# tamthuc1995/ImageRestoration-Development-Unrolling

Measured on AMD Instinct MI355X. Metric: MPix/sec + PSNR@σ=25, 10-stage GGTV-GGLR on 256×256 patches, 1/2/4/8 GPU, higher is better.
Workload: dtype f32; 1 GPU; MultiScaleGraphFilter (image-domain GGTV-GGLR, v13 feature CNN) G=32 F=3 C=96, S=10 stages, 256x256 RGB sigma=25, weights: trained fixture; global_batch=64, per_gpu_batch=64, image=256x256x3, parallelism=batch-sharded x1, no collective in the data path

## Files before the change

imagerestoration-development-unrolling_amd/_native.py:

```python
from __future__ import annotations

import ctypes
import os
from ctypes import c_int, c_int64, c_void_p

HERE = os.path.dirname(os.path.abspath(__file__))
LIB_PATH = os.environ.get("GRR_LIB", os.path.join(HERE, "libgrr.so"))


class NativeUnavailable(RuntimeError):
    """libgrr.so could not be loaded (build it with build_native.py)."""


class GrrError(RuntimeError):

    def __init__(self, fn: str, status: int, msg: str):
        super().__init__(f"{fn} failed (status {status}): {msg}")
        self.status = status


STATUS_NAMES = {0: "GRR_OK", 1: "GRR_ERR_INVALID_ARG", 2: "GRR_ERR_SHAPE", 3: "GRR_ERR_UNSUPPORTED", 4: "GRR_ERR_HIP"}


class Stencil(ctypes.Structure):
    _fields_ = [("p01", c_void_p), ("p02a", c_void_p), ("p02b", c_void_p), ("p03", c_void_p)]


P = c_void_p
I = c_int
L = c_int64
Fl = ctypes.c_float

SIGNATURES = {
    "grr_version": [],
    "grr_last_error": [],
    "grr_set_kernel_variant": [I],
    "grr_lnb_set_phases": [I],
    "grr_lnb_rep_fused": [I, I, I, I],
    "grr_set_scratch_allocator": [P, P, P],
    "grr_release_scratch": [],
    "grr_scratch_bytes": [],
    "grr_neighbor_table": [P, I, I, P],
    "grr_stream_copy": [P, P, L, P],
    "grr_edge_weights": [P, L, P, P, P, I, I, I, I, I, P],
    "grr_gtv_pair_weights": [P, P, I, I, I, I, P],
    "grr_edge_weights_block": [P, L, I, P, I, P, P, P, P, I, I, I, I, I, P],
    "grr_pool2": [P, P, I, I, I, I, P],
    "grr_system_half": [P, P, P, Stencil, Stencil, P, P, P, I, I, I, I, I, P],
    "grr_gtv_rhs_half": [P, P, Stencil, I, P, P, I, I, I, I, I, P],
    "grr_gtv_rhs_full": [P, P, P, Stencil, I, P, P, P, P, P, P, I, I, I, I, I, P],
    "grr_gtv_rhs_full_rep": [P, I, P, I, P, Stencil, I, P, P, P, P, P, P, I, I, I, I, I, P],
    "grr_system_step": [P, P, P, P, P, P, Stencil, Stencil, P, P, P, P, P, P, P, P, P, I, I, I, I, I, P],
    "grr_system_step2": [P, P, P, P, P, P, Stencil, Stencil, P, P, P, P, Stencil, Stencil, P, P, P, P, P, P, P, P,
                         P, P, P, I, I, I, I, I, P],
    "grr_system_first_pair": [P, P, P, I, P, P, P, Stencil, Stencil, P, P, P, P, P, P, Stencil, Stencil, P, P, P, P, P,
                              P, P, P, P, I, I, I, I, I, P],
    "grr_system_step2_train": [P, P, P, P, P, P, Stencil, Stencil, P, P, P, P, Stencil, Stencil, P, P, P, P, P, P,
                               P, P, P, P, P, P, I, I, I, I, I, P],
    "grr_glr_stage": [P, P, P, P, Stencil, P, P, P, P, P, I, I, I, I, I, P],
    "grr_conv1x1": [P, P, P, I, I, I, L, P],
    "grr_conv1x1_workspace_bytes": [I, I],
    "grr_conv1x1_ws": [P, P, P, P, I, I, I, L, P],
    "grr_conv2x2s2": [P, P, P, I, I, I, I, I, P],
    "grr_conv3x3_embed_supported": [I, I],
    "grr_conv3x3_embed": [P, P, P, I, I, I, I, I, P],
    "grr_conv3x3_embed_bwd_w_workspace_bytes": [I, I, I, I, I],
    "grr_conv3x3_embed_bwd_w": [P, P, P, P, I, I, I, I, I, P],
    "grr_conv3x3_embed_bwd_x": [P, P, P, I, I, I, I, I, P],
    "grr_convt2x2s2_workspace_bytes": [I, I, I, I, I],
    "grr_convt2x2s2": [P, P, P, P, I, I, I, I, I, P],
    "grr_conv1x1_cat2_supported": [I, I, I, L],
    "grr_conv1x1_cat2_workspace_bytes": [I, I, I],
    "grr_conv1x1_cat2": [P, P, P, P, P, I, I, I, I, L, P],
    "grr_ffn_workspace_bytes": [I, I, I, I, I],
    "grr_ffn_forward": [P, P, P, P, P, P, P, P, I, I, I, I, I, P],
    "grr_wgrad_workspace_bytes": [I, I, I, L],
    "grr_wgrad_set_tiles": [I],
    "grr_wgrad": [P, P, P, P, I, I, I, L, P],
    "grr_lnb_workspace_bytes": [I, I, I, I, I],
    "grr_lnb_forward": [P, P, P, P, P, P, P, P, I, I, I, I, I, P],
    "grr_lnb_forward_keep": [P, P, P, P, P, P, P, P, I, I, I, I, I, P],
    "grr_lnb_forward_c8": [P, P, P, P, P, P, P, P, I, I, I, I, I, I, P],
    "grr_c8_convert": [P, P, I, I, I, I, I, P],
    "grr_feature_edges_supported": [I, I, I, I, I],
    "grr_feature_edges_workspace_bytes": [I],
    "grr_feature_edges": [P, I, P, P, P, P, P, P, P, I, I, I, I, I, I, P],
    "grr_lnb_fused": [I, I],
    "grr_lnb_fused_workspace_bytes": [I, I],
    "grr_lnb_set_fused": [I],
    "grr_dw3_ring_check": [I],
    "grr_repeat_graphs": [P, P, I, I, I, L, P],
    "grr_lnb_forward_rep": [P, I, I, P, P, P, P, P, P, P, P, I, I, I, I, P],
    "grr_neighbor_gather": [P, P, I, I, I, I, P],
    "grr_normalize_features": [P, P, P, I, I, I, I, I, P],
    "grr_stats_conv": [P, Stencil, I, P, I, I, I, I, I, P],
    "grr_glr_op_l_norm": [P, P, P, I, I, I, I, I, P],
    "grr_gtv_op_c": [P, P, Stencil, P, I, I, I, I, I, P],
    "grr_gtv_op_c_transpose": [P, P, Stencil, P, P, I, I, I, I, I, P],
    "grr_neighbor_gather_bwd": [P, P, I, I, I, I, P],
    "grr_normalize_features_bwd": [P, P, P, P, P, I, I, I, I, I, P],
    "grr_stats_conv_bwd": [P, Stencil, I, P, P, P, I, I, I, I, I, P],
    "grr_glr_op_l_norm_bwd": [P, P, P, P, P, I, I, I, I, I, P],
    "grr_gtv_op_c_bwd": [P, P, Stencil, P, P, P, P, P, I, I, I, I, I, P],
    "grr_gtv_op_c_transpose_bwd": [P, P, Stencil, P, P, P, P, P, P, I, I, I, I, I, P],
    "grr_bwd_stencil": [P, P, I, P, I, P, I, I, I, I, I, P],
    "grr_bwd_tapgrad": [P, P, I, P, P, I, I, I, I, I, P],
    "grr_bwd_padj2": [P, P, P, P, P, P, P, I, I, I, I, I, P],
    "grr_bwd_glr": [P, P, P, P, Fl, P, P, P, P, I, I, I, I, I, P],
    "grr_bwd_pair": [P, P, P, P, Fl, P, P, P, P, I, I, I, I, I, P],
    "grr_bwd_prox": [P, P, P, P, P, Fl, P, P, P, P, P, I, I, I, I, I, P],
    "grr_bwd_set_term_rows": [I],
    "grr_bwd_set_term_tail": [I],
    "grr_bwd_set_term_acc_max_w": [I],
    "grr_lnb_set_bwd_ring": [I],
    "grr_bwd_term_fused": [I, P, P, P, P, P, P, Fl, P, P, P, P, P, I, I, I, I, I, P],
    "grr_bwd_term_acc_supported": [I, I, I, I],
    "grr_bwd_term_fused_acc": [I, P, P, P, P, P, P, Fl, P, P, P, P, P, I, I, I, I, I, P],
    "grr_bwd_pair_weights": [P, P, P, I, I, I, I, P],
    "grr_bwd_edge_weights": [P, L, P, P, P, P, L, P, I, I, I, I, I, P],
    "grr_bwd_graph_dot": [P, P, Fl, P, I, I, I, I, I, P],
    "grr_bwd_lincomb": [P, P, P, P, P, I, I, I, I, I, I, P],
    "grr_bwd_cg_glue": [P, P, P, P, P, P, P, P, P, P, P, P, P, P, P, P, P, P, I, I, I, I, I, P],
    "grr_bwd_cg_glue_pool": [P, P, P, P, P, P, P, P, P, P, P, P, P, P, P, P, P, P, P, I, I, I, I, I, P],
    "grr_bwd_unpool2_acc": [P, P, I, I, I, I, P],
    "grr_conv2x2s2_bwd_data": [P, P, P, I, I, I, I, I, P],
    "grr_interleave2x2": [P, P, I, I, I, I, P],
    "grr_lnb_norm": [P, P, P, P, I, I, L, P],
    "grr_lnb_norm_bwd": [P, P, P, P, P, P, I, I, L, P],
    "grr_lnb_norm_bwd_skip": [P, P, P, P, P, P, P, P, P, I, I, L, P],
    "grr_dwconv3": [P, P, P, I, I, I, I, P],
    "grr_dwconv3_bwd": [P, P, P, P, P, I, I, I, I, P],
    "grr_lnb_gate": [P, P, P, P, I, I, L, P],
    "grr_lnb_gate_bwd_scaled": [P, P, P, P, P, I, I, L, P],
    "grr_lnb_gate_dw3_bwd": [P, P, P, P, P, P, P, P, I, I, I, I, P],
    "grr_lnb_dw3_gate": [P, P, P, I, I, I, I, P],
    "grr_ffn_dw3_gate": [P, P, P, I, I, I, I, P],
    "grr_ffn_gate_dw3_bwd": [P, P, P, P, P, P, P, I, I, I, I, P],
    "grr_win_edge_weights": [P, L, P, P, I, P, P, I, I, I, I, I, P],
    "grr_win_solver": [I, P, I, P, P, P, P, P, P, P, P, P, P, P, P, I, P, P, I, I, I, I, I, P],
    "grr_win_mix": [P, P, P, P, I, I, I, I, I, P],
    "grr_win_pair_weights": [P, P, I, P, I, I, I, I, P],
    "grr_win_bwd_stencil": [P, P, I, P, I, P, I, I, I, I, I, P],
    "grr_win_bwd_tapgrad": [P, P, I, P, P, I, I, I, I, I, P],
    "grr_win_bwd_glr": [P, P, P, P, I, P, Fl, P, P, P, P, P, I, I, I, I, I, P],
    "grr_win_bwd_gtv": [P, P, P, P, I, I, P, P, Fl, P, P, P, P, P, P, I, I, I, I, I, P],
    "grr_win_bwd_gather": [P, P, P, I, P, P, I, I, I, I, I, P],
    "grr_win_bwd_gather_fused": [P, P, P, P, I, I, I, P, P, P, P, I, I, I, I, I, P],
    "grr_win_bwd_edge_weights": [P, L, P, P, P, P, I, P, L, P, I, I, I, I, I, P],
    "grr_win_bwd_mix": [P, P, P, P, P, I, I, I, I, I, P],
    "grr_image_io_supported": [I, I, I],
    "grr_tile_gather": [P, I, I, I, I, P, I, I, I, P, P],
    "grr_tile_scatter": [P, P, I, I, I, P, I, I, I, I, P],
    "grr_u8_sse": [P, P, L, P, P],
}
_RESTYPES = {"grr_version": c_int, "grr_last_error": ctypes.c_char_p, "grr_lnb_workspace_bytes": c_int64,
             "grr_conv1x1_workspace_bytes": c_int64, "grr_wgrad_workspace_bytes": c_int64,
             "grr_ffn_workspace_bytes": c_int64, "grr_scratch_bytes": c_int64,
             "grr_lnb_fused_workspace_bytes": c_int64, "grr_feature_edges_workspace_bytes": c_int64,
             "grr_conv3x3_embed_bwd_w_workspace_bytes": c_int64, "grr_conv1x1_cat2_workspace_bytes": c_int64, "grr_convt2x2s2_workspace_bytes": c_int64}

_lib = None


def load() -> ctypes.CDLL:
    global _lib
    if _lib is not None:
        return _lib
    if not os.path.exists(LIB_PATH):
        raise NativeUnavailable(
            f"{LIB_PATH} not found: build it with `python imagerestoration-development-unrolling_amd/build_native.py`")
    try:
        lib = ctypes.CDLL(LIB_PATH)
    except OSError as e:
        raise NativeUnavailable(f"cannot load {LIB_PATH}: {e}") from e
    for name, argtypes in SIGNATURES.items():
        fn = getattr(lib, name)
        fn.argtypes = argtypes
        fn.restype = _RESTYPES.get(name, c_int)
    _register_scratch_allocator(lib)
    _lib = lib
    return lib


_SCRATCH_ALLOC_FN = ctypes.CFUNCTYPE(c_void_p, ctypes.c_uint64, c_int, c_void_p, c_void_p)
_SCRATCH_FREE_FN = ctypes.CFUNCTYPE(None, c_void_p, c_int, c_void_p, c_void_p)


def _scratch_alloc(nbytes, device, stream, _ctx):
    try:
        import torch
        return int(torch.cuda.caching_allocator_alloc(int(nbytes), device, int(stream or 0)))
    except Exception:
        return None


def _scratch_free(ptr, _device, _stream, _ctx):
    try:
        import torch
        torch.cuda.caching_allocator_delete(int(ptr))
    except Exception:
        pass


_scratch_cbs = (_SCRATCH_ALLOC_FN(_scratch_alloc), _SCRATCH_FREE_FN(_scratch_free))


def _register_scratch_allocator(lib) -> None:
    st = lib.grr_set_scratch_allocator(ctypes.cast(_scratch_cbs[0], c_void_p), ctypes.cast(_scratch_cbs[1], c_void_p),
                                       None)
    if st != 0:
        raise NativeUnavailable(f"grr_set_scratch_allocator failed: {lib.grr_last_error()!r}")


def release_scratch() -> None:
    import torch
    torch.cuda.synchronize()
    call("grr_release_scratch")


def call(name: str, *args) -> None:
    lib = load()
    st = getattr(lib, name)(*args)
    if st != 0:
        msg = lib.grr_last_error()
        raise GrrError(name, st, (msg or b"").decode(errors="replace"))
```

imagerestoration-development-unrolling_amd/csrc/feature_ops.hip:

```cpp
#include "grr_common.h"

namespace grr {

typedef float f32x16 __attribute__((ext_vector_type(16)));

constexpr int GT = 256;
constexpr int BM = 128, BN = 128, BK = 16;
constexpr int APAD = BM + 2;
constexpr int BPAD = BN + 4;

enum { LD_PLAIN = 0, LD_LN = 1, LD_IM2COL = 2 };
enum { EP_STORE = 0, EP_SKIP = 1 };

struct GemmArgs {
  const float* x;
  const float* wt;
  const float* ln_sd;
  const float* ln_w;
  const float* res;
  const float* skip;
  float* out;
  int K, M;
  int64_t P;
  int Hin, Win, Wo;
// ... 766 lines not shown
}

int64_t grr_conv1x1_cat2_workspace_bytes(int Ka, int Kb, int M) {
  if (Ka < 1 || Kb < 1) return 0;
  return grr_conv1x1_workspace_bytes(Ka + Kb, M);
}

grr_status grr_conv1x1_cat2(const float* xa, const float* xb, const float* wt, float* out, void* workspace, int B,
                            int Ka, int Kb, int M, int64_t P, void* stream) {
  clear_error();
  GRR_REQUIRE(xa && xb && wt && out && workspace && B > 0 && Ka > 0 && Kb > 0 && M > 0 && P > 0, GRR_ERR_INVALID_ARG,
              "grr_conv1x1_cat2: bad args");
  GRR_REQUIRE(out != xa && out != xb, GRR_ERR_INVALID_ARG, "grr_conv1x1_cat2: out aliases an input");
  GRR_REQUIRE(((uintptr_t)workspace & 255) == 0, GRR_ERR_INVALID_ARG, "grr_conv1x1_cat2: workspace not 256-B aligned");
  GRR_REQUIRE(grr_conv1x1_cat2_supported(Ka, Kb, M, P), GRR_ERR_UNSUPPORTED,
              "grr_conv1x1_cat2: Ka=%d (a multiple of 16), Kb=%d, M=%d, P=%lld not supported", Ka, Kb, M, (long long)P);
  hipStream_t s = (hipStream_t)stream;
  const int K = Ka + Kb, KS = (K + 15) / 16, nch = (M + X3_MCH - 1) / X3_MCH;
  uint16_t* frag = (uint16_t*)workspace;
  const int64_t nf = (int64_t)nch * x3_chunk_bytes(KS) / 2;
  hipLaunchKernelGGL(x3_pack_kernel, dim3((unsigned)std::min<int64_t>((nf + 255) / 256, 1 << 16)), dim3(256), 0, s,
                     wt, nullptr, frag, M, K, KS, nch);
  grr_status st = launch_status("grr_conv1x1_cat2/pack");
  if (st != GRR_OK) return st;
  if (K > 128)
    return launch_x3k<X3K_STORE, true>(xa, frag, out, B, K, M, P, s, "grr_conv1x1_cat2", nullptr, nullptr, nullptr, xb,
                                       Ka);
  return launch_x3<false, true>(xa, frag, out, B, K, M, P, s, "grr_conv1x1_cat2", xb, Ka);
}

grr_status grr_conv2x2s2(const float* x, const float* wt, float* out, int B, int K, int M, int H, int W,
                         void* stream) {
  clear_error();
  GRR_REQUIRE(x && wt && out && B > 0 && K > 0 && M > 0 && H > 1 && W > 1, GRR_ERR_INVALID_ARG,
              "grr_conv2x2s2: bad args");
  GemmArgs a{};
  a.x = x; a.wt = wt; a.out = out; a.K = 4 * K; a.M = M; a.P = (int64_t)(H / 2) * (W / 2);
  a.Hin = H; a.Win = W; a.Wo = W / 2;
  return launch_gemm<LD_IM2COL, EP_STORE>(a, B, (hipStream_t)stream, "grr_conv2x2s2");
}

}

namespace grr {

struct FfnLayout {
  int64_t sd, h, g, f1, f2, total;
  int KS1, nch1, KS2, nch2;
};
static int64_t a64(int64_t n) { return (n + 63) / 64 * 64; }
static FfnLayout ffn_layout(int B, int C, int hid, int64_t P) {
  FfnLayout L{};
  L.KS1 = (C + 15) / 16; L.nch1 = (2 * hid + 31) / 32;
  L.KS2 = (hid + 15) / 16; L.nch2 = (C + 31) / 32;
  L.sd = 0;
  L.h = a64((int64_t)B * P);
  L.g = L.h + a64((int64_t)B * 2 * hid * P);
  L.f1 = L.g + a64((int64_t)B * hid * P);
  L.f2 = L.f1 + a64((int64_t)L.nch1 * x3_chunk_bytes(L.KS1) / 4);
  L.total = L.f2 + a64((int64_t)L.nch2 * x3_chunk_bytes(L.KS2) / 4);
  return L;
}

template <bool FFN>
static grr_status block_x3_forward(const float* x, const float* ln_w, const float* w_in, const float* w_dw,
                                   const float* w_out, const float* skip, float* out, float* ws, int B, int C,
                                   int hid, int H, int W, hipStream_t s) {
  const int64_t P = (int64_t)H * W;
  const FfnLayout L = ffn_layout(B, C, hid, P);
  float* sd = ws + L.sd;
  float* hbuf = ws + L.h;
  float* gbuf = ws + L.g;
  uint16_t* f1 = reinterpret_cast<uint16_t*>(ws + L.f1);
  uint16_t* f2 = reinterpret_cast<uint16_t*>(ws + L.f2);
  auto pack = [&](const float* w, const float* lw, uint16_t* frag, int M, int K, int KS, int nch) {
    const int64_t nf = (int64_t)nch * x3_chunk_bytes(KS) / 2;
    hipLaunchKernelGGL(x3_pack_kernel, dim3((unsigned)std::min<int64_t>((nf + 255) / 256, 1 << 16)), dim3(256), 0, s,
                       w, lw, frag, M, K, KS, nch);
    return launch_status("grr_ffn_forward/pack");
  };
  grr_status st = pack(w_in, ln_w, f1, 2 * hid, C, L.KS1, L.nch1);
  if (st != GRR_OK) return st;
  st = pack(w_out, nullptr, f2, C, hid, L.KS2, L.nch2);
  if (st != GRR_OK) return st;
  if (C <= 128) {
    st = launch_x3<true>(x, f1, hbuf, B, C, 2 * hid, P, s, "grr_ffn_forward/w_in");
  } else {
    GRR_REQUIRE((int64_t)B * ((P + 63) / 64) < (1ll << 31), GRR_ERR_UNSUPPORTED, "grr_ffn_forward: grid too large");
    hipLaunchKernelGGL(ln_stats_kernel, dim3((unsigned)((int64_t)B * ((P + 63) / 64))), dim3(64 * LN_G), 0, s, x, sd,
                       B, C, P);
    st = launch_status("grr_ffn_forward/ln_stats");
    if (st != GRR_OK) return st;
    st = launch_x3k<X3K_LN>(x, f1, hbuf, B, C, 2 * hid, P, s, "grr_ffn_forward/w_in", sd);
  }
  if (st != GRR_OK) return st;
  const int tx = (W + DT - 1) / DT, ty = (H + DT - 1) / DT;
  const uint64_t nb = (uint64_t)B * hid * tx * ty;
  GRR_REQUIRE(nb < (1ull << 31), GRR_ERR_UNSUPPORTED, "grr_ffn_forward: grid too large");
  hipLaunchKernelGGL(dw_gate_kernel<FFN>, dim3((unsigned)nb), dim3(256), 0, s, hbuf, w_dw, gbuf, hid, H, W, tx, ty,
                     (uint32_t)nb);
  st = launch_status("grr_ffn_forward/dw_gate");
  if (st != GRR_OK) return st;
  return launch_x3k<X3K_SKIP>(gbuf, f2, out, B, hid, C, P, s, "grr_ffn_forward/w_out", nullptr, x, skip);
}

}

extern "C" {

int64_t grr_lnb_workspace_bytes(int B, int C, int hid, int H, int W) {
  if (B <= 0 || C <= 0 || hid <= 0 || H <= 0 || W <= 0) return 0;
  const int64_t f = C <= 128 ? grr::lnb_mfma_workspace_floats(B, C, hid, H, W)
                             : grr::ffn_layout(B, C, hid, (int64_t)H * W).total;
  return f * (int64_t)sizeof(float);
}

int64_t grr_lnb_fused_workspace_bytes(int C, int hid) {
  if (!grr::lnb_fused(C, hid)) return 0;
  return grr::fused_pack_floats(C, hid) * (int64_t)sizeof(float);
}

grr_status grr_lnb_forward(const float* x, const float* ln_w, const float* w1, const float* wdw, const float* w2,
                           const float* skip, float* out, void* workspace, int B, int C, int hid, int H, int W,
                           void* stream) {
  grr::clear_error();
  GRR_REQUIRE(x && ln_w && w1 && wdw && w2 && skip && out && workspace && B > 0 && C > 1 && hid > 0 && H > 0 &&
                  W > 0,
              GRR_ERR_INVALID_ARG, "grr_lnb_forward: bad args");
  GRR_REQUIRE(out != x, GRR_ERR_INVALID_ARG, "grr_lnb_forward: out aliases x");
  GRR_REQUIRE(((uintptr_t)workspace & 255) == 0, GRR_ERR_INVALID_ARG, "grr_lnb_forward: workspace not 256-B aligned");
  hipStream_t s = (hipStream_t)stream;
  if (C <= 128)
    return grr::lnb_forward_mfma(x, ln_w, w1, wdw, w2, skip, out, (float*)workspace, B, C, hid, H, W, s);
  GRR_REQUIRE(C <= 4096 && hid <= 4096, GRR_ERR_UNSUPPORTED, "grr_lnb_forward: C=%d, hid=%d > 4096", C, hid);
  return grr::block_x3_forward<false>(x, ln_w, w1, wdw, w2, skip, out, (float*)workspace, B, C, hid, H, W, s);
}

grr_status grr_lnb_forward_c8(const float* x, const float* ln_w, const float* w1, const float* wdw, const float* w2,
                              const float* skip, float* out, void* workspace, int B, int C, int hid, int H, int W,
                              int layout, void* stream) {
  grr::clear_error();
  GRR_REQUIRE(x && ln_w && w1 && wdw && w2 && skip && out && workspace && B > 0 && C > 1 && hid > 0 && H > 0 &&
                  W > 0 && layout >= 0 && layout <= 3,
              GRR_ERR_INVALID_ARG, "grr_lnb_forward_c8: bad args");
  GRR_REQUIRE(out != x, GRR_ERR_INVALID_ARG, "grr_lnb_forward_c8: out aliases x");
  GRR_REQUIRE(((uintptr_t)workspace & 255) == 0 && ((uintptr_t)x & 15) == 0 && ((uintptr_t)out & 15) == 0,
              GRR_ERR_INVALID_ARG, "grr_lnb_forward_c8: workspace 256-B, x and out 16-B aligned");
  GRR_REQUIRE(grr_lnb_fused(C, hid) && (int64_t)((C + 7) / 8) * 8 * H * W * 4 < (1ll << 31), GRR_ERR_UNSUPPORTED,
              "grr_lnb_forward_c8: needs the fused pass (grr_lnb_fused) and 2^31 bytes per blocked image");
  return grr::lnb_forward_mfma(x, ln_w, w1, wdw, w2, skip, out, (float*)workspace, B, C, hid, H, W,
                               (hipStream_t)stream, false, layout);
}

namespace grr {
__global__ __launch_bounds__(256) void c8_pack_kernel(const float* __restrict__ x, float* __restrict__ y, int C, int64_t HW,
                                                     int64_t n) {
  for (int64_t i = blockIdx.x * (int64_t)blockDim.x + threadIdx.x; i < n; i += (int64_t)gridDim.x * blockDim.x) {
    const int64_t p = i % HW, r = i / HW;
    const int nb = (C + 7) / 8, blk = (int)(r % nb);
    const int64_t b = r / nb;
    float v[8];
#pragma unroll
    for (int j = 0; j < 8; ++j) {
      const int c = 8 * blk + j;
      v[j] = c < C ? x[(b * C + c) * HW + p] : 0.f;
    }
    float4* o = reinterpret_cast<float4*>(y + i * 8);
    o[0] = make_float4(v[0], v[1], v[2], v[3]);
    o[1] = make_float4(v[4], v[5], v[6], v[7]);
  }
}
__global__ __launch_bounds__(256) void c8_unpack_kernel(const float* __restrict__ y, float* __restrict__ x, int C,
                                                       int64_t HW, int64_t n) {
  for (int64_t i = blockIdx.x * (int64_t)blockDim.x + threadIdx.x; i < n; i += (int64_t)gridDim.x * blockDim.x) {
    const int64_t p = i % HW, r = i / HW;
    const int nb = (C + 7) / 8, blk = (int)(r % nb);
    const int64_t b = r / nb;
#pragma unroll
    for (int j = 0; j < 8; ++j) {
      const int c = 8 * blk + j;
      if (c < C) x[(b * C + c) * HW + p] = y[i * 8 + j];
    }
  }
}
}

grr_status grr_c8_convert(const float* src, float* dst, int B, int C, int H, int W, int to_blocked, void* stream) {
  grr::clear_error();
  GRR_REQUIRE(src && dst && src != dst && B > 0 && C > 0 && H > 0 && W > 0 && ((uintptr_t)(to_blocked ? dst : src) & 15) == 0,
              GRR_ERR_INVALID_ARG, "grr_c8_convert: bad args (the blocked tensor 16-B aligned)");
  const int64_t HW = (int64_t)H * W, n = (int64_t)B * ((C + 7) / 8) * HW;
  const unsigned grid = (unsigned)std::min<int64_t>((n + 255) / 256, 65536);
  if (to_blocked)
    hipLaunchKernelGGL(grr::c8_pack_kernel, dim3(grid), dim3(256), 0, (hipStream_t)stream, src, dst, C, HW, n);
  else
    hipLaunchKernelGGL(grr::c8_unpack_kernel, dim3(grid), dim3(256), 0, (hipStream_t)stream, src, dst, C, HW, n);
  return grr::launch_status("grr_c8_convert");
}

grr_status grr_lnb_forward_keep(const float* x, const float* ln_w, const float* w1, const float* wdw,
                                const float* w2, const float* skip, float* out, void* workspace, int B, int C,
                                int hid, int H, int W, void* stream) {
  grr::clear_error();
  GRR_REQUIRE(x && ln_w && w1 && wdw && w2 && skip && out && workspace && B > 0 && C > 1 && hid > 0 && H > 0 &&
                  W > 0,
              GRR_ERR_INVALID_ARG, "grr_lnb_forward_keep: bad args");
  GRR_REQUIRE(out != x, GRR_ERR_INVALID_ARG, "grr_lnb_forward_keep: out aliases x");
  GRR_REQUIRE(((uintptr_t)workspace & 255) == 0, GRR_ERR_INVALID_ARG,
              "grr_lnb_forward_keep: workspace not 256-B aligned");
  GRR_REQUIRE(C <= 128, GRR_ERR_UNSUPPORTED, "grr_lnb_forward_keep: C=%d > 128", C);
  return grr::lnb_forward_mfma(x, ln_w, w1, wdw, w2, skip, out, (float*)workspace, B, C, hid, H, W,
                               (hipStream_t)stream, true);
}

grr_status grr_lnb_forward_rep(const float* src, int Cs, int R, const float* x, const float* ln_w, const float* w1,
                               const float* wdw, const float* w2, const float* skip, float* out, void* workspace,
                               int B, int hid, int H, int W, void* stream) {
  grr::clear_error();
  GRR_REQUIRE(src && ln_w && w1 && wdw && w2 && skip && out && workspace && B > 0 && Cs > 0 && R > 0 &&
                  hid > 0 && H > 0 && W > 0,
              GRR_ERR_INVALID_ARG, "grr_lnb_forward_rep: bad args");
  GRR_REQUIRE(out != x && out != src, GRR_ERR_INVALID_ARG, "grr_lnb_forward_rep: out aliases an input");
  GRR_REQUIRE(((uintptr_t)workspace & 255) == 0, GRR_ERR_INVALID_ARG,
              "grr_lnb_forward_rep: workspace not 256-B aligned");
  GRR_REQUIRE(R * Cs <= 128, GRR_ERR_UNSUPPORTED, "grr_lnb_forward_rep: R*Cs=%d > 128", R * Cs);
  return grr::lnb_forward_mfma_rep(src, Cs, R, x, ln_w, w1, wdw, w2, skip, out, (float*)workspace, B, hid, H, W,
                                   (hipStream_t)stream);
}

int64_t grr_ffn_workspace_bytes(int B, int C, int hid, int H, int W) {
  if (B <= 0 || C <= 1 || hid <= 0 || H <= 0 || W <= 0) return 0;
  return grr::ffn_layout(B, C, hid, (int64_t)H * W).total * (int64_t)sizeof(float);
}

grr_status grr_ffn_forward(const float* x, const float* ln_w, const float* w_in, const float* w_dw, const float* w_out,
                           const float* skip, float* out, void* workspace, int B, int C, int hid, int H, int W,
                           void* stream) {
  grr::clear_error();
  GRR_REQUIRE(x && ln_w && w_in && w_dw && w_out && skip && out && workspace && B > 0 && C > 1 && hid > 0 &&
                  H > 0 && W > 0,
              GRR_ERR_INVALID_ARG, "grr_ffn_forward: bad args");
  GRR_REQUIRE(out != x, GRR_ERR_INVALID_ARG, "grr_ffn_forward: out aliases x");
  GRR_REQUIRE(((uintptr_t)workspace & 255) == 0, GRR_ERR_INVALID_ARG, "grr_ffn_forward: workspace not 256-B aligned");
  GRR_REQUIRE(C <= 4096 && hid <= 4096, GRR_ERR_UNSUPPORTED, "grr_ffn_forward: C=%d, hid=%d > 4096", C, hid);
  return grr::block_x3_forward<true>(x, ln_w, w_in, w_dw, w_out, skip, out, (float*)workspace, B, C, hid, H, W,
                                     (hipStream_t)stream);
}

grr_status grr_repeat_graphs(const float* img, float* out, int B, int Cin, int G, int64_t P, void* stream) {
  clear_error();
  GRR_REQUIRE(img && out && B > 0 && Cin > 0 && G > 0 && P > 0, GRR_ERR_INVALID_ARG, "grr_repeat_graphs: bad args");
  const int64_t n = (int64_t)B * Cin * P;
  if (P % 4 == 0 && (uintptr_t)img % 16 == 0 && (uintptr_t)out % 16 == 0) {
    const int64_t nq = n / 4;
    const int blocks = (int)std::min<int64_t>((nq + 255) / 256, 1 << 16);
    hipLaunchKernelGGL(repeat_graphs_kernel, dim3(blocks), dim3(256), 0, (hipStream_t)stream, img, out, Cin, G, P, nq);
  } else {
    const int blocks = (int)std::min<int64_t>((n + 255) / 256, 1 << 16);
    hipLaunchKernelGGL(repeat_graphs_scalar_kernel, dim3(blocks), dim3(256), 0, (hipStream_t)stream, img, out, Cin,
                       G, P, n);
  }
  return launch_status("grr_repeat_graphs");
}

}
```

imagerestoration-development-unrolling_amd/csrc/grr_common.h:

```cpp
#pragma once

#include <hip/hip_runtime.h>
#include <stdint.h>

#include <cstdio>
#include <string>

#include "../../include/grr.h"

namespace grr {

void set_error(const char* fmt, ...);
void clear_error();

#define GRR_REQUIRE(cond, code, ...)        \
  do {                                      \
    if (!(cond)) {                          \
      ::grr::set_error(__VA_ARGS__);        \
      return code;                          \
    }                                       \
  } while (0)

grr_status launch_status(const char* what);

constexpr int kWave = 64;
constexpr int kXcd = 8;

__device__ __forceinline__ uint32_t xcd_remap(uint32_t bid, uint32_t n) {
  const uint32_t xcd = bid % kXcd, q = n / kXcd, r = n % kXcd;
  const uint32_t base = xcd < r ? xcd * (q + 1) : r * (q + 1) + (xcd - r) * q;
  return base + bid / kXcd;
}

int64_t lnb_mfma_workspace_floats(int B, int C, int hid, int H, int W);
int64_t fused_pack_floats(int C, int hid);
bool lnb_fused(int C, int hid);
bool lnb_fused(int C, int hid);
grr_status lnb_forward_mfma(const float* x, const float* ln_w, const float* w1, const float* wdw, const float* w2,
                            const float* skip, float* out, float* ws, int B, int C, int hid, int H, int W,
                            hipStream_t s, bool keep_g = false, int io = 0);
grr_status lnb_forward_mfma_rep(const float* xh, int Ch, int R, const float* x, const float* ln_w, const float* w1,
                                const float* wdw, const float* w2, const float* skip, float* out, float* ws, int B,
                                int hid, int H, int W, hipStream_t s);

__device__ __forceinline__ int clampi(int v, int lo, int hi) { return v < lo ? lo : (v > hi ? hi : v); }

struct Red {
  float* p;
  uint32_t nslot;
};
__device__ __forceinline__ void red_put(const Red& r, int idx, uint32_t slot, float v) {
  if (r.p) r.p[(size_t)idx * r.nslot + slot] = v;
}

class RedScratch {
 public:
  static constexpr int kMax = 4;
  explicit RedScratch(hipStream_t s) : s_(s) {}
  RedScratch(const RedScratch&) = delete;
  RedScratch& operator=(const RedScratch&) = delete;
  ~RedScratch();
  int plan(float* dst, int n, uint32_t nslot);
  grr_status alloc(const char* what);
  Red red(int i) const { return Red{dst_[i] ? part_[i] : nullptr, nslot_[i]}; }
  grr_status finish(const char* what);

 private:
  hipStream_t s_;
  int k_ = 0;
  float* dst_[kMax] = {};
  float* part_[kMax] = {};
  int n_[kMax] = {};
  uint32_t nslot_[kMax] = {};
  void* base_ = nullptr;
};

}
```

imagerestoration-development-unrolling_amd/csrc/lnb_ops.hip:

```cpp
#include <cstdlib>

#include "grr_common.h"

namespace grr {

typedef float f32x2 __attribute__((ext_vector_type(2)));
typedef float f32x4 __attribute__((ext_vector_type(4)));
typedef float f32x16 __attribute__((ext_vector_type(16)));
typedef __bf16 bf16x8 __attribute__((ext_vector_type(8)));
typedef __attribute__((address_space(3))) void* lds_ptr_t;

__device__ __forceinline__ void split3x8(const float (&v)[8], bf16x8& t0, bf16x8& t1, bf16x8& t2) {
#pragma unroll
  for (int j = 0; j < 8; ++j) {
    const __bf16 h0 = (__bf16)v[j];
    const float r1 = v[j] - (float)h0;
    const __bf16 h1 = (__bf16)r1;
    const float r2 = r1 - (float)h1;
    t0[j] = h0;
    t1[j] = h1;
    t2[j] = (__bf16)r2;
  }
}
__host__ __device__ inline uint16_t bf16_bits_rne(float v) {
// ... 772 lines not shown
#pragma unroll
      for (int t = 0; t < MT; ++t) acc2[t] *= f;
    }
    E = eg;
    const int Eu = E == 1000 ? 0 : E;
    f16x8 gh, gl;
#pragma unroll
    for (int q = 0; q < 8; ++q) {
      const float v = ldexpf(gq[q], Eu);
      const _Float16 h0 = (_Float16)v;
      gh[q] = h0;
      gl[q] = (_Float16)(v - (float)h0);
    }
    const float* slot = cslot + lane * 4;
#pragma unroll
    for (int t = 0; t < MT; ++t) {
      const f16x8 ah = *reinterpret_cast<const f16x8*>(slot + (4 + 2 * t + 0) * 256);
      const f16x8 al = *reinterpret_cast<const f16x8*>(slot + (4 + 2 * t + 1) * 256);
      acc2[t] = __builtin_amdgcn_mfma_f32_32x32x16_f16(al, gh, acc2[t], 0, 0, 0);
      acc2[t] = __builtin_amdgcn_mfma_f32_32x32x16_f16(ah, gl, acc2[t], 0, 0, 0);
      acc2[t] = __builtin_amdgcn_mfma_f32_32x32x16_f16(ah, gh, acc2[t], 0, 0, 0);
    }
  };

  for (int c = 0; c < nch; ++c) {
    asm volatile("s_waitcnt vmcnt(%0)" ::"i"(DPW) : "memory");
    __builtin_amdgcn_s_barrier();
    asm volatile("" ::: "memory");
    issue(c + 3);
    gate_gemm2(c, gemm1(c));
  }
  asm volatile("s_waitcnt vmcnt(0)" ::: "memory");

  const float* rs2 = smem + ((nch - 1) % LR_NSLOT) * SLOTF + CI * 256 + 32;
  const float s0 = a.skip[0], s1 = a.skip[1] * ldexpf(1.0f, E == 1000 ? 0 : -E);
  const __amdgpu_buffer_rsrc_t ors = __builtin_amdgcn_make_buffer_rsrc(a.out + (int64_t)b * C * P, 0,
                                                                        (int)((int64_t)C * P * 4), 0x00020000);
  float xo[CS];
#pragma unroll
  for (int c = 0; c < CS; ++c) xo[c] = xb[(int64_t)c * P + pc];
  const uint32_t vb = p < P ? (uint32_t)(4 * kh * P + p) * 4u : 0x80000000u;
#pragma unroll
  for (int t = 0; t < MT; ++t)
#pragma unroll
    for (int i = 0; i < 16; ++i) {
      const int m0 = 32 * t + (i & 3) + 8 * (i >> 2);
      const float xv = kh ? xo[(m0 + 4) % CS] : xo[m0 % CS];
      const float r2 = rs2[min(m0 + 4 * kh, C - 1)];
      const uint32_t vo = m0 + 4 < C ? vb : (m0 < C && !kh ? vb : 0x80000000u);
      __builtin_amdgcn_raw_buffer_store_b32(__float_as_uint(s0 * xv + s1 * (acc2[t][i] * r2)), ors, vo, m0 * P * 4, 0);
    }
}

constexpr int LF_TW = 32;
constexpr int LF_TH = 8;
constexpr int LF_HWD = LF_TW + 2;
constexpr int LF_HR = LF_TH + 2;
constexpr int LF_NQ = LF_HWD * LF_HR;
constexpr int LF_NBLK = (LF_NQ + 31) / 32;
constexpr int LF_PP = 2 * LF_NBLK * 32;
constexpr int LF_HBUF = 16 * LF_PP;
constexpr int LF_NSLOT = 3;
constexpr int LF_XE = 10;
constexpr int LF_DSTR = 36;
constexpr int LF_TAPS = 8 * LF_DSTR;
__host__ __device__ constexpr int fused_images(int KS, int MT) { return 2 * KS + 2 * MT + 2; }

struct LnbFusedArgs {
  const float* x;
  const char* pack;
  const float* r2;
  const float* skip;
  float* out;
  float* g;
  float var_den;
  int C, hid, H, W, tiles_x, tiles_y, nch, ntiles;
};

__global__ void lnb_fused_pack_kernel(const float* __restrict__ w1, const float* __restrict__ ln_w,
                                      const float* __restrict__ wdw, const float* __restrict__ w2,
                                      char* __restrict__ pack, float* __restrict__ r2, int C, int hid, int KS,
                                      int MT, int nch) {
  const int NI = fused_images(KS, MT);
  const int64_t n_img = (int64_t)nch * NI * 256;
  const int64_t n = n_img + C;
  for (int64_t i = blockIdx.x * (int64_t)blockDim.x + threadIdx.x; i < n; i += (int64_t)gridDim.x * blockDim.x) {
    if (i >= n_img) {
      const int m = (int)(i - n_img);
      r2[m] = ldexpf(1.0f, -rep_w2_exp(w2, m, hid));
      continue;
    }
    const int64_t img = i >> 8;
    const int e = (int)(i & 255), c = (int)(img / NI), im = (int)(img % NI), l = e >> 2;
    uint32_t word = 0;
    if (im < 2 * KS) {
      const int q = im & 1, s = im >> 1, r = l & 31, pj = 16 * c + (r >> 1);
      if (pj < hid) {
        const int row = (r & 1 ? hid : 0) + pj;
        const int sc = head16_row_exp(w1, ln_w, row, C, 1);
        float v[2];
#pragma unroll
        for (int u = 0; u < 2; ++u) {
          const int k = 16 * s + 8 * (l >> 5) + 2 * (e & 3) + u;
          v[u] = k < C ? ldexpf(w1[(int64_t)row * C + k] * ln_w[k], sc) : 0.f;
        }
        word = f16_pair_word(v[0], v[1], q);
      }
    } else if (im < 2 * KS + 2 * MT) {
      const int t = (im - 2 * KS) >> 1, q = (im - 2 * KS) & 1, m = 32 * t + (l & 31);
      if (m < C) {
        const int sc = rep_w2_exp(w2, m, hid);
        float v[2];
#pragma unroll
        for (int u = 0; u < 2; ++u) {
          const int pj = 16 * c + 8 * (l >> 5) + 2 * (e & 3) + u;
          v[u] = pj < hid ? ldexpf(w2[(int64_t)m * hid + pj], sc) : 0.f;
        }
        word = f16_pair_word(v[0], v[1], q);
      }
    } else {
      const int r = (im - 2 * KS - 2 * MT) * 256 + e;
      if (r < LF_TAPS) {
        const int w = 2 * (r / LF_DSTR) + ((r >> 1) & 1), t = (r % LF_DSTR) >> 2, comp = r & 1, pj = 16 * c + w;
        if (pj < hid && t < 9) {
          const int row = (comp ? hid : 0) + pj;
          const float fold = comp ? -0.69314718055994531f : -1.44269504088896341f;
          word = __float_as_uint(ldexpf(wdw[(int64_t)row * 9 + t], -(head16_row_exp(w1, ln_w, row, C, 1) + LF_XE)) *
                                 fold);
        }
      }
    }
    reinterpret_cast<uint32_t*>(pack)[i] = word;
  }
}

typedef uint32_t u32x4 __attribute__((ext_vector_type(4)));
typedef __attribute__((address_space(4))) const float* const_f32_t;
typedef float f32x2v __attribute__((ext_vector_type(2)));
typedef _Float16 f16x2 __attribute__((ext_vector_type(2)));
__device__ __forceinline__ void split2_f16(float a, float b, uint32_t& hi, uint32_t& lo) {
  const f32x2v v = f32x2v{a, b};
  const f16x2 h = __builtin_convertvector(v, f16x2);
  const f16x2 l = __builtin_convertvector(v - __builtin_convertvector(h, f32x2v), f16x2);
  hi = __builtin_bit_cast(uint32_t, h);
  lo = __builtin_bit_cast(uint32_t, l);
}

#ifndef GRR_FUSED_DIAG
#define GRR_FUSED_DIAG 0
#endif
#ifndef GRR_FUSED_STAMP
#define GRR_FUSED_STAMP 0
#endif
#if GRR_FUSED_STAMP
__device__ unsigned long long g_fused_stamps[1024 * 8 * 8];
#define FSTAMP(k)                                              \
  do {                                                         \
    const unsigned long long t_ = __builtin_amdgcn_s_memtime(); \
    st_acc[k] += t_ - st_prev;                                 \
    st_prev = t_;                                              \
  } while (0)
#else
#define FSTAMP(k) \
  do {            \
  } while (0)
#endif

struct FusedTile {
  int b, y0, x0;
};
__device__ __forceinline__ FusedTile fused_tile(const LnbFusedArgs& a, int t) {
  const int tx = t % a.tiles_x, r = t / a.tiles_x;
  return FusedTile{r / a.tiles_y, (r % a.tiles_y) * LF_TH, tx * LF_TW};
}

template <int KS, int MT, int IO>
__global__ __launch_bounds__(512, 1) void lnb_fused16_kernel(LnbFusedArgs a) {
  constexpr bool IN8 = (IO & 1) != 0, OUT8 = (IO & 2) != 0;
  constexpr int NI = fused_images(KS, MT), SLOTF = NI * 256;
  constexpr int DPW = (NI + 7) / 8;
  __shared__ __attribute__((aligned(16))) float smem[2 * LF_HBUF + LF_NSLOT * SLOTF + 32 * MT];
  float* const ring = smem + 2 * LF_HBUF;
  float* const r2s = ring + LF_NSLOT * SLOTF;

  const int tid = threadIdx.x, lane = tid & 63, kh = lane >> 5;
  const int wave = __builtin_amdgcn_readfirstlane(tid >> 6);
  const int H = a.H, W = a.W, C = a.C, hid = a.hid, nch = a.nch;
  if (tid < 32 * MT) r2s[tid] = tid < C ? a.r2[tid] : 0.f;
  const int HW = H * W;
  const int G = gridDim.x, wg = blockIdx.x;
  const int my_tiles = wg < a.ntiles ? (a.ntiles - wg + G - 1) / G : 0;
  const int nsteps = my_tiles * nch;

  auto issue = [&](int sl, int chunk) {
    int sv = __builtin_amdgcn_readfirstlane(sl), cv = __builtin_amdgcn_readfirstlane(chunk), wv = wave;
    asm volatile("" : "+s"(sv), "+s"(cv), "+s"(wv));
    float* slot = ring + sv * SLOTF;
    const char* src = a.pack + (int64_t)cv * NI * 1024 + lane * 16;
#pragma unroll
    for (int i = 0; i < DPW; ++i) {
      const int img = min(i * 8 + wv, NI - 1);
      dma16_opaque(src + img * 1024, slot + img * 256);
    }
  };
  int dch = nch > 1 ? 1 : 0, dsl = 1;
  auto advance_dma = [&]() {
    dch = dch + 1 == nch ? 0 : dch + 1;
    dsl = dsl == LF_NSLOT - 1 ? 0 : dsl + 1;
  };
  if (nsteps == 0) return;
#if GRR_FUSED_STAMP
  unsigned long long st_acc[8] = {}, st_prev = __builtin_amdgcn_s_memtime();
  auto stamp_out = [&]() {
    if (lane < 8 && blockIdx.x < 1024) {
      unsigned long long v = 0;
#pragma unroll
      for (int k = 0; k < 8; ++k) v = lane == k ? st_acc[k] : v;
      g_fused_stamps[(blockIdx.x * 8 + wave) * 8 + lane] = v;
    }
  };
#endif
  issue(0, 0);
  asm volatile("s_waitcnt vmcnt(0)" ::: "memory");
  __builtin_amdgcn_s_barrier();
  asm volatile("" ::: "memory");

  if (wave < 4) {
    constexpr int NBW = (LF_NBLK + 3) / 4;
    const bool has_last = wave + 4 * (NBW - 1) < LF_NBLK;
    f16x8 xh[NBW][KS], xl[NBW][KS];
    float corr[NBW];
    bool wave_corr = false;
    int c = 0, tile = wg, sl = 0;
    for (int i = 0; i <= nsteps; ++i) {
      issue(dsl, dch);
      advance_dma();
      FSTAMP(0);
      if (i < nsteps && !(GRR_FUSED_DIAG & 2)) {
        if (c == 0) {
          const FusedTile T = fused_tile(a, tile);
          const int cx = IN8 ? 8 * ((C + 7) / 8) : C;
          const __amdgpu_buffer_rsrc_t xr = __builtin_amdgcn_make_buffer_rsrc(
              const_cast<float*>(a.x + (int64_t)T.b * cx * HW), 0, (int)((int64_t)cx * HW * 4), 0x00020000);
          bool any_corr = false;
#pragma unroll
          for (int k = 0; k < NBW; ++k) {
            const int q = min((wave + 4 * k) * 32 + (lane & 31), LF_NQ - 1);
            const int hy = q / LF_HWD, hx = q - hy * LF_HWD;
            const int gy = clampi(T.y0 - 1 + hy, 0, H - 1), gx = clampi(T.x0 - 1 + hx, 0, W - 1);
            const int vo = (8 * kh * HW + gy * W + gx) * 4;
            int hw4 = HW * 4;
            asm volatile("" : "+s"(hw4));
            float xv[KS][8];
            if constexpr (IN8) {
              const uint32_t vo8 = (uint32_t)((kh * HW + gy * W + gx) * 32);
#pragma unroll
              for (int s = 0; s < KS; ++s) {
                const u32x4 lo = __builtin_bit_cast(u32x4, __builtin_amdgcn_raw_buffer_load_b128(xr, vo8, 16 * s * hw4, 0));
                const u32x4 hi = __builtin_bit_cast(u32x4, __builtin_amdgcn_raw_buffer_load_b128(xr, vo8 + 16, 16 * s * hw4, 0));
#pragma unroll
                for (int j = 0; j < 4; ++j) {
                  xv[s][j] = __uint_as_float(lo[j]);
                  xv[s][4 + j] = __uint_as_float(hi[j]);
                }
              }
            } else {
#pragma unroll
              for (int s = 0; s < KS; ++s)
#pragma unroll
                for (int j = 0; j < 8; ++j)
                  xv[s][j] = __uint_as_float(__builtin_amdgcn_raw_buffer_load_b32(xr, vo, (16 * s + j) * hw4, 0));
            }
            float sum = 0.f;
#pragma unroll
            for (int s = 0; s < KS; ++s)
#pragma unroll
              for (int j = 0; j < 8; ++j) sum += xv[s][j];
            sum += __shfl_xor(sum, 32);
            const float mean = sum / (float)C;
            float sq = 0.f;
#pragma unroll
            for (int s = 0; s < KS; ++s)
#pragma unroll
              for (int j = 0; j < 8; ++j) {
                const float d = 16 * s + 8 * kh + j < C ? xv[s][j] - mean : 0.f;
                sq += d * d;
              }
            sq += __shfl_xor(sq, 32);
            const float rstd = 1.0f / sqrtf(sq / a.var_den + 1e-5f);
            float mx = 0.f;
#pragma unroll
            for (int s = 0; s < KS; ++s)
#pragma unroll
              for (int j = 0; j < 8; ++j) {
                xv[s][j] *= rstd;
                mx = fmaxf(mx, fabsf(xv[s][j]));
              }
            mx = fmaxf(mx, __shfl_xor(mx, 32));
            int ep = LF_XE;
            if (mx != 0.f) {
              int e;
              frexpf(mx, &e);
              if (e > 14 - LF_XE || e < -LF_XE) ep = clampi(14 - e, -100, 100);
            }
            corr[k] = ldexpf(1.0f, LF_XE - ep);
            any_corr |= ep != LF_XE;
#pragma unroll
            for (int s = 0; s < KS; ++s) {
              uint32_t hw[4], lw[4];
#pragma unroll
              for (int j = 0; j < 4; ++j)
                split2_f16(ldexpf(xv[s][2 * j], ep), ldexpf(xv[s][2 * j + 1], ep), hw[j], lw[j]);
              xh[k][s] = __builtin_bit_cast(f16x8, u32x4{hw[0], hw[1], hw[2], hw[3]});
              xl[k][s] = __builtin_bit_cast(f16x8, u32x4{lw[0], lw[1], lw[2], lw[3]});
            }
          }
          wave_corr = __builtin_amdgcn_readfirstlane((int)__any(any_corr)) != 0;
        }
        FSTAMP(1);
        const float* slot = ring + sl * SLOTF + lane * 4;
        f32x16 acc[NBW];
#pragma unroll
        for (int k = 0; k < NBW; ++k) acc[k] = f32x16{};
        f16x8 ah = *reinterpret_cast<const f16x8*>(slot);
        f16x8 al = *reinterpret_cast<const f16x8*>(slot + 256);
#pragma unroll
        for (int s = 0; s < KS; ++s) {
          f16x8 bh, bl;
          if (s + 1 < KS) {
            bh = *reinterpret_cast<const f16x8*>(slot + (2 * s + 2) * 256);
            bl = *reinterpret_cast<const f16x8*>(slot + (2 * s + 3) * 256);
          }
#pragma unroll
          for (int k = 0; k < NBW; ++k) {
            if (k == NBW - 1 && !has_last) continue;
            acc[k] = __builtin_amdgcn_mfma_f32_32x32x16_f16(al, xh[k][s], acc[k], 0, 0, 0);
            acc[k] = __builtin_amdgcn_mfma_f32_32x32x16_f16(ah, xl[k][s], acc[k], 0, 0, 0);
            acc[k] = __builtin_amdgcn_mfma_f32_32x32x16_f16(ah, xh[k][s], acc[k], 0, 0, 0);
          }
          if (s + 1 < KS) {
            ah = bh;
            al = bl;
          }
          __builtin_amdgcn_sched_barrier(0);
        }
        FSTAMP(2);
        float* hb = smem + (i & 1) * LF_HBUF;
#pragma unroll
        for (int k = 0; k < NBW; ++k) {
          if (k == NBW - 1 && !has_last) continue;
          if (wave_corr) acc[k] *= corr[k];
          const int q = (wave + 4 * k) * 32 + (lane & 31);
#pragma unroll
          for (int u = 0; u < 4; ++u)
            *reinterpret_cast<f32x4*>(hb + (2 * u + kh) * 2 * LF_PP + 4 * q) =
                f32x4{acc[k][4 * u], acc[k][4 * u + 1], acc[k][4 * u + 2], acc[k][4 * u + 3]};
        }
        if (++c == nch) {
          c = 0;
          tile += G;
        }
        sl = sl == LF_NSLOT - 1 ? 0 : sl + 1;
      }
      FSTAMP(3);
      asm volatile("s_waitcnt vmcnt(0) lgkmcnt(0)" ::: "memory");
      FSTAMP(4);
      __builtin_amdgcn_s_barrier();
      asm volatile("" ::: "memory");
      FSTAMP(5);
    }
#if GRR_FUSED_STAMP
    stamp_out();
#endif
    return;
  }

  __builtin_amdgcn_s_setprio(1);
  const int cw = wave - 4;
  const int col = lane & 31;
  f32x16 acc2[2][MT];
  int E[2] = {1000, 1000};
  int ch = 0, ctile = wg, csl = 0;
  for (int i = 0; i <= nsteps; ++i) {
    issue(dsl, dch);
    advance_dma();
    FSTAMP(0);
    if (i >= 1 && !(GRR_FUSED_DIAG & 1)) {
      const int st = i - 1;
      if (ch == 0) {
#pragma unroll
        for (int rb = 0; rb < 2; ++rb) {
#pragma unroll
          for (int t = 0; t < MT; ++t) acc2[rb][t] = f32x16{};
          E[rb] = 1000;
        }
      }
      const float* slot = ring + csl * SLOTF;
      const FusedTile T = fused_tile(a, ctile);
      const int gxo = T.x0 + col;
      const float* w2s = slot + 2 * KS * 256 + lane * 4;
      float g[2][8];
      const float* hwin4 = smem + (st & 1) * LF_HBUF + 4 * kh * 2 * LF_PP + 4 * (2 * cw * LF_HWD + col);
      const float* tapd = slot + (2 * KS + 2 * MT) * 256 + 4 * kh * LF_DSTR;
      f32x4 tc[4][9], wc[4][12];
      auto ld_taps = [&](int dd, int r) __attribute__((always_inline)) {
#pragma unroll
        for (int x = 0; x < 3; ++x) tc[dd][3 * r + x] = *reinterpret_cast<const f32x4*>(tapd + dd * LF_DSTR + 4 * (3 * r + x));
      };
      auto ld_row = [&](int dd, int r) __attribute__((always_inline)) {
#pragma unroll
        for (int x = 0; x < 3; ++x)
          wc[dd][3 * r + x] = *reinterpret_cast<const f32x4*>(hwin4 + dd * 2 * LF_PP + 4 * (r * LF_HWD + x));
      };
      auto gate2 = [&](const f32x4& mv, int rb, int dd) __attribute__((always_inline)) {
#pragma unroll
        for (int e = 0; e < 2; ++e) {
          const float m = mv[2 * e], v = mv[2 * e + 1];
          g[rb][2 * dd + e] = (GRR_FUSED_DIAG & 8) ? (m * v) : (m * v) * __builtin_amdgcn_rcpf(1.0f + __builtin_amdgcn_exp2f(m));
        }
      };
      ld_taps(0, 0);
      ld_row(0, 0);
      ld_row(0, 1);
#pragma unroll
      for (int dd = 0; dd < 4; ++dd) {
        f32x4 mv0, mv1;
        ld_taps(dd, 1);
        ld_row(dd, 2);
        __builtin_amdgcn_sched_barrier(0);
        mv0 = tc[dd][0] * wc[dd][0];
        mv1 = tc[dd][0] * wc[dd][3];
#pragma unroll
        for (int x = 1; x < 3; ++x) {
          mv0 = __builtin_elementwise_fma(tc[dd][x], wc[dd][x], mv0);
          mv1 = __builtin_elementwise_fma(tc[dd][x], wc[dd][3 + x], mv1);
        }
        __builtin_amdgcn_sched_barrier(0);
        ld_taps(dd, 2);
        ld_row(dd, 3);
        __builtin_amdgcn_sched_barrier(0);
#pragma unroll
        for (int x = 0; x < 3; ++x) {
          mv0 = __builtin_elementwise_fma(tc[dd][3 + x], wc[dd][3 + x], mv0);
          mv1 = __builtin_elementwise_fma(tc[dd][3 + x], wc[dd][6 + x], mv1);
        }
        __builtin_amdgcn_sched_barrier(0);
        if (dd < 3) {
          ld_taps(dd + 1, 0);
          ld_row(dd + 1, 0);
          ld_row(dd + 1, 1);
        }
        __builtin_amdgcn_sched_barrier(0);
#pragma unroll
        for (int x = 0; x < 3; ++x) {
          mv0 = __builtin_elementwise_fma(tc[dd][6 + x], wc[dd][6 + x], mv0);
          mv1 = __builtin_elementwise_fma(tc[dd][6 + x], wc[dd][9 + x], mv1);
        }
        gate2(mv0, 0, dd);
        gate2(mv1, 1, dd);
        __builtin_amdgcn_sched_barrier(0);
      }
      FSTAMP(1);
      if (a.g) {
        float* gb = a.g + (int64_t)T.b * hid * HW;
#pragma unroll
        for (int rb = 0; rb < 2; ++rb) {
          const int yy = T.y0 + 2 * cw + rb;
          if (yy < H && gxo < W) {
#pragma unroll
            for (int jj = 0; jj < 8; ++jj) {
              const int pj = 16 * ch + 8 * kh + jj;
              if (pj < hid) gb[(int64_t)pj * HW + yy * W + gxo] = g[rb][jj];
            }
          }
        }
      }
#pragma unroll
      for (int rb = 0; rb < 2; ++rb) {
        float gm = 0.f;
#pragma unroll
        for (int jj = 0; jj < 8; ++jj) gm = fmaxf(gm, fabsf(g[rb][jj]));
        const auto gs = __builtin_amdgcn_permlane32_swap(__float_as_uint(gm), __float_as_uint(gm), false, false);
        gm = fmaxf(__uint_as_float(gs[0]), __uint_as_float(gs[1]));
        int eg = E[rb];
        if (gm != 0.f) {
          int e;
          frexpf(gm, &e);
          eg = min(E[rb], clampi(14 - e, -100, 100));
        }
        if (__builtin_amdgcn_readfirstlane((int)__any(eg != E[rb] && E[rb] != 1000)) != 0) {
          const float f = E[rb] != 1000 ? ldexpf(1.0f, eg - E[rb]) : 1.0f;
#pragma unroll
          for (int t = 0; t < MT; ++t) acc2[rb][t] *= f;
        }
        E[rb] = eg;
        const int Eu = eg == 1000 ? 0 : eg;
        f16x8 gh, gl;
#pragma unroll
        for (int jj = 0; jj < 8; ++jj) {
          const float v = ldexpf(g[rb][jj], Eu);
          const _Float16 h0 = (_Float16)v;
          gh[jj] = h0;
          gl[jj] = (_Float16)(v - (float)h0);
        }
#pragma unroll
        for (int t = 0; t < MT; ++t) {
          const f16x8 ah = *reinterpret_cast<const f16x8*>(w2s + (2 * t + 0) * 256);
          const f16x8 al = *reinterpret_cast<const f16x8*>(w2s + (2 * t + 1) * 256);
          acc2[rb][t] = __builtin_amdgcn_mfma_f32_32x32x16_f16(al, gh, acc2[rb][t], 0, 0, 0);
          acc2[rb][t] = __builtin_amdgcn_mfma_f32_32x32x16_f16(ah, gl, acc2[rb][t], 0, 0, 0);
          acc2[rb][t] = __builtin_amdgcn_mfma_f32_32x32x16_f16(ah, gh, acc2[rb][t], 0, 0, 0);
        }
      }
      FSTAMP(2);
      if (ch == nch - 1) {
        const float s0 = a.skip[0], s1 = a.skip[1];
        const int c8 = 8 * ((C + 7) / 8);
        const int cx = IN8 ? c8 : C, co = OUT8 ? c8 : C;
        const __amdgpu_buffer_rsrc_t xrs = __builtin_amdgcn_make_buffer_rsrc(
            const_cast<float*>(a.x + (int64_t)T.b * cx * HW), 0, (int)((int64_t)cx * HW * 4), 0x00020000);
        const __amdgpu_buffer_rsrc_t ors = __builtin_amdgcn_make_buffer_rsrc(a.out + (int64_t)T.b * co * HW, 0,
                                                                              (int)((int64_t)co * HW * 4), 0x00020000);
        const int Eb[2] = {E[0], E[1]};
#pragma unroll
        for (int rb = 0; rb < 2; ++rb) {
          const float sc = s1 * ldexpf(1.0f, Eb[rb] == 1000 ? 0 : -Eb[rb]);
#pragma unroll
          for (int t = 0; t < MT; ++t)
#pragma unroll
            for (int u = 0; u < 16; ++u) acc2[rb][t][u] *= sc * r2s[32 * t + (u & 3) + 8 * (u >> 2) + 4 * kh];
        }
        __builtin_amdgcn_sched_barrier(0);
        int hw4 = __builtin_amdgcn_readfirstlane(HW * 4);
        asm volatile("" : "+s"(hw4));
        uint32_t vx[2], vo[2], vx8[2], vo8[2];
#pragma unroll
        for (int rb = 0; rb < 2; ++rb) {
          const int yy = T.y0 + 2 * cw + rb;
          const uint32_t pix = (uint32_t)(min(yy, H - 1) * W + min(gxo, W - 1));
          const bool in = yy < H && gxo < W;
          vx[rb] = (uint32_t)(4 * kh * HW + pix) * 4u;
          vo[rb] = in ? vx[rb] : 0x80000000u;
          vx8[rb] = pix * 32u + 16u * kh;
          vo8[rb] = in ? vx8[rb] : 0x80000000u;
        }
        float xv[2][MT][16];
#pragma unroll
        for (int rb = 0; rb < 2; ++rb)
#pragma unroll
          for (int t = 0; t < MT; ++t) {
            if constexpr (IN8) {
#pragma unroll
              for (int q = 0; q < 4; ++q) {
                const u32x4 v = __builtin_bit_cast(
                    u32x4, __builtin_amdgcn_raw_buffer_load_b128(xrs, vx8[rb], (4 * t + q) * 8 * hw4, 0));
#pragma unroll
                for (int r = 0; r < 4; ++r) xv[rb][t][4 * q + r] = __uint_as_float(v[r]);
              }
            } else {
#pragma unroll
              for (int u = 0; u < 16; ++u)
                xv[rb][t][u] = __uint_as_float(
                    __builtin_amdgcn_raw_buffer_load_b32(xrs, vx[rb], (32 * t + (u & 3) + 8 * (u >> 2)) * hw4, 0));
            }
          }
#pragma unroll
        for (int rb = 0; rb < 2; ++rb)
#pragma unroll
          for (int t = 0; t < MT; ++t) {
            if constexpr (OUT8) {
#pragma unroll
              for (int q = 0; q < 4; ++q) {
                u32x4 v;
#pragma unroll
                for (int r = 0; r < 4; ++r) v[r] = __float_as_uint(s0 * xv[rb][t][4 * q + r] + acc2[rb][t][4 * q + r]);
                __builtin_amdgcn_raw_buffer_store_b128(__builtin_bit_cast(decltype(__builtin_amdgcn_raw_buffer_load_b128(
                                                           ors, 0, 0, 0)), v),
                                                       ors, vo8[rb], (4 * t + q) * 8 * hw4, 0);
              }
            } else {
#pragma unroll
              for (int u = 0; u < 16; ++u)
                __builtin_amdgcn_raw_buffer_store_b32(__float_as_uint(s0 * xv[rb][t][u] + acc2[rb][t][u]), ors, vo[rb],
                                                      (32 * t + (u & 3) + 8 * (u >> 2)) * hw4, 0);
            }
          }
      }
      if (++ch == nch) {
        ch = 0;
        ctile += G;
      }
      csl = csl == LF_NSLOT - 1 ? 0 : csl + 1;
    }
    FSTAMP(3);
    asm volatile("s_waitcnt vmcnt(0) lgkmcnt(0)" ::: "memory");
    FSTAMP(4);
    __builtin_amdgcn_s_barrier();
    asm volatile("" ::: "memory");
    FSTAMP(5);
  }
#if GRR_FUSED_STAMP
  stamp_out();
#endif
}

#if GRR_FUSED_STAMP
extern "C" int grr_lnb_fused_stamps(unsigned long long* host, int n) {
  return hipMemcpyFromSymbol(host, HIP_SYMBOL(g_fused_stamps), sizeof(unsigned long long) * std::min(n, 1024 * 64),
                             0, hipMemcpyDeviceToHost) == hipSuccess ? 0 : 1;
}
#endif

constexpr int LM_NBB = 2;
constexpr int LM_PX = 4 * LM_NBB * 32;
constexpr int LM_KD = 16;

struct LnbMixArgs {
  const float* g;
  const char* w2f;
  const float* x;
  int xs_c;
  const float* skip;
  float* out;
  int64_t P;
  int C, hid, KS2, tiles;
  uint32_t nblk;
};

__global__ void lnb_w2_pack_kernel(const float* __restrict__ w2, uint16_t* __restrict__ frag, int C, int hid,
                                   int MT, int KS2) {
  const int64_t n = (int64_t)KS2 * MT * 3 * 512;
  for (int64_t i = blockIdx.x * (int64_t)blockDim.x + threadIdx.x; i < n; i += (int64_t)gridDim.x * blockDim.x) {
    const int j = (int)(i & 7), l = (int)((i >> 3) & 63);
    const int64_t img = i >> 9;
    const int q = (int)(img % 3), t = (int)((img / 3) % MT), s = (int)(img / (3 * MT));
    const int m = 32 * t + (l & 31), k = 16 * s + 8 * (l >> 5) + j;
    frag[i] = (m < C && k < hid) ? split_term(w2[(int64_t)m * hid + k], q) : (uint16_t)0;
  }
}

template <int MT, bool V4>
__global__ __launch_bounds__(256, MT >= 4 ? 1 : 2) void lnb_mix_kernel(LnbMixArgs a) {
  constexpr int NI = MT * 3;
  constexpr int WPW = (NI + 3) / 4;
  constexpr int GPW = V4 ? LM_KD / 4 : LM_KD;
  constexpr int DPW = WPW + GPW;
  constexpr int WF = NI * 256;
  constexpr int SLOTF = WF + LM_KD * LM_PX;
  constexpr int NSLOT = 3;
  __shared__ __attribute__((aligned(16))) float smem[NSLOT * SLOTF];

  const int tid = threadIdx.x, lane = tid & 63;
  const int wave = __builtin_amdgcn_readfirstlane(tid >> 6);
  const uint32_t lb = xcd_remap(blockIdx.x, a.nblk);
  const int b = lb / a.tiles, tile = lb - b * a.tiles;
  const int64_t P = a.P;
  const int C = a.C, hid = a.hid, KS2 = a.KS2;
  const int r = lane & 31, hh = lane >> 5;
  const int64_t p0 = (int64_t)tile * LM_PX;

  const float* gb = a.g + (int64_t)b * hid * P;
  const int64_t gcol = V4 ? min(p0 + 4 * lane, P - 4) : 0;
  auto issue = [&](int s) {
    const int ss = min(s, KS2 - 1);
    float* slot = smem + (s % NSLOT) * SLOTF;
    const char* src = a.w2f + (int64_t)ss * NI * 1024 + lane * 16;
#pragma unroll
    for (int i = 0; i < WPW; ++i) {
      const int img = min(i * 4 + wave, NI - 1);
      dma16(src + img * 1024, slot + img * 256);
    }
    float* gs = slot + WF;
#pragma unroll
    for (int i = 0; i < GPW; ++i) {
      if constexpr (V4) {
        const int kr = wave * GPW + i;
        const int k = min(LM_KD * ss + kr, hid - 1);
        dma16(gb + (int64_t)k * P + gcol, gs + kr * LM_PX);
      } else {
        const int kr = wave * 4 + (i >> 2), part = i & 3;
        const int k = min(LM_KD * ss + kr, hid - 1);
        const int64_t pc = min(p0 + part * 64 + lane, P - 1);
        __builtin_amdgcn_global_load_lds(gb + (int64_t)k * P + pc, (lds_ptr_t)(gs + kr * LM_PX + part * 64), 4, 0,
                                         0);
      }
    }
  };

  f32x16 acc[MT][LM_NBB];
#pragma unroll
  for (int t = 0; t < MT; ++t)
#pragma unroll
    for (int nb = 0; nb < LM_NBB; ++nb) acc[t][nb] = f32x16{};

  issue(0);
  issue(1);
  for (int s = 0; s < KS2; ++s) {
    asm volatile("s_waitcnt vmcnt(%0)" ::"i"(DPW) : "memory");
    __builtin_amdgcn_s_barrier();
    issue(s + 2);
    const float* slot = smem + (s % NSLOT) * SLOTF;
    const float* gs = slot + WF + (8 * hh) * LM_PX + wave * LM_NBB * 32 + r;
    bf16x8 bq[LM_NBB][3];
#pragma unroll
    for (int nb = 0; nb < LM_NBB; ++nb) {
      float gv[8];
#pragma unroll
      for (int j = 0; j < 8; ++j) gv[j] = gs[j * LM_PX + nb * 32];
      split3x8(gv, bq[nb][0], bq[nb][1], bq[nb][2]);
    }
    const float* ws = slot + lane * 4;
#pragma unroll
    for (int t = 0; t < MT; ++t) {
      const bf16x8 a0 = *reinterpret_cast<const bf16x8*>(ws + (3 * t + 0) * 256);
      const bf16x8 a1 = *reinterpret_cast<const bf16x8*>(ws + (3 * t + 1) * 256);
      const bf16x8 a2 = *reinterpret_cast<const bf16x8*>(ws + (3 * t + 2) * 256);
#pragma unroll
      for (int nb = 0; nb < LM_NBB; ++nb)
        GRR_X3_MFMA(__builtin_amdgcn_mfma_f32_32x32x16_bf16, acc[t][nb], a0, a1, a2, bq[nb][0], bq[nb][1],
                    bq[nb][2]);
    }
  }
  asm volatile("s_waitcnt vmcnt(0)" ::: "memory");

  const float s0 = a.skip[0], s1 = a.skip[1];
  const int img_bytes = (int)((int64_t)C * P * 4);
  const int XC = a.xs_c > 0 ? a.xs_c : C;
  const __amdgpu_buffer_rsrc_t xrs = __builtin_amdgcn_make_buffer_rsrc(
      const_cast<float*>(a.x + (int64_t)b * XC * P), 0, (int)((int64_t)XC * P * 4), 0x00020000);
  const __amdgpu_buffer_rsrc_t ors = __builtin_amdgcn_make_buffer_rsrc(a.out + (int64_t)b * C * P, 0, img_bytes,
                                                                        0x00020000);
  const int Pi = (int)P;
#pragma unroll
  for (int nb = 0; nb < LM_NBB; ++nb) {
    const int p = (int)p0 + (wave * LM_NBB + nb) * 32 + r;
    const int pc = min(p, Pi - 1);
#pragma unroll
    for (int t = 0; t < MT; ++t) {
      float xv[16];
#pragma unroll
      for (int i = 0; i < 16; ++i) {
        const int m = min(32 * t + (i & 3) + 8 * (i >> 2) + 4 * hh, C - 1);
        const int mx = XC == C ? m : m % XC;
        xv[i] = __uint_as_float(__builtin_amdgcn_raw_buffer_load_b32(xrs, (mx * Pi + pc) * 4, 0, 0));
      }
#pragma unroll
      for (int i = 0; i < 16; ++i) {
        const int m = 32 * t + (i & 3) + 8 * (i >> 2) + 4 * hh;
        const uint32_t off = (m < C && p < Pi) ? (uint32_t)(m * Pi + p) * 4u : 0x80000000u;
        __builtin_amdgcn_raw_buffer_store_b32(__float_as_uint(s0 * xv[i] + s1 * acc[t][nb][i]), ors, off, 0, 0);
      }
    }
  }
}

static int head_ks(int C) { return (C + 31) / 32; }
static int head_nb(int KS) { return KS <= 3 ? 4 : 3; }
static int64_t align64(int64_t n) { return (n + 63) / 64 * 64; }
static int head16_ks(int C) { return (C + 15) / 16; }
static bool head16_enabled(int C) { return head16_ks(C) <= 6; }
static int64_t head_pack_floats(int C, int hid) {
  const int64_t bf = (int64_t)((hid + LH_JC - 1) / LH_JC) * head_images(head_ks(C)) * 256;
  const int64_t f16 = (int64_t)((hid + L6_NP - 1) / L6_NP) * head16_images(head16_ks(C)) * 256;
  return align64(std::max(bf, f16));
}
static int64_t mix_pack_floats(int C, int hid) {
  return align64((int64_t)((hid + LM_KD - 1) / LM_KD) * ((C + 31) / 32) * 3 * 256);
}

int g_lnb_fused_on = 1;
bool lnb_fused(int C, int hid) { return g_lnb_fused_on && C >= 2 && C <= 96 && hid >= 1; }
int64_t fused_pack_floats(int C, int hid) {
  const int KS = (C + 15) / 16, MT = (C + 31) / 32, nch = (hid + 15) / 16;
  return align64((int64_t)nch * fused_images(KS, MT) * 256) + align64(C);
}

int64_t lnb_mfma_workspace_floats(int B, int C, int hid, int H, int W) {
  const int64_t two_kernel = align64((int64_t)B * hid * H * W) +
                             std::max(head_pack_floats(C, hid) + mix_pack_floats(C, hid), fused_pack_floats(C, hid));
  const int64_t rep = align64((int64_t)((hid + 15) / 16) * rep_images((C + 31) / 32) * 256);
  return std::max(two_kernel, rep);
}

template <int KS, int NB>
static void launch_head(const LnbHeadArgs& h, hipStream_t s) {
  hipLaunchKernelGGL((lnb_head_kernel<KS, NB>), dim3(h.nblk), dim3(512), 0, s, h);
}
template <int KS>
static void launch_head16(const LnbHeadArgs& h, hipStream_t s) {
  hipLaunchKernelGGL((lnb_head16_kernel<KS, 8>), dim3(h.nblk), dim3(512), 0, s, h);
}
template <int MT>
static void launch_mix(const LnbMixArgs& m, bool v4, hipStream_t s) {
  if (v4) hipLaunchKernelGGL((lnb_mix_kernel<MT, true>), dim3(m.nblk), dim3(256), 0, s, m);
  else hipLaunchKernelGGL((lnb_mix_kernel<MT, false>), dim3(m.nblk), dim3(256), 0, s, m);
}

int g_lnb_phases = 7;

template <int KS>
static void launch_fused(const LnbFusedArgs& f, unsigned grid, int io, hipStream_t s) {
  switch (io) {
    case 1: hipLaunchKernelGGL((lnb_fused16_kernel<KS, (KS + 1) / 2, 1>), dim3(grid), dim3(512), 0, s, f); break;
    case 2: hipLaunchKernelGGL((lnb_fused16_kernel<KS, (KS + 1) / 2, 2>), dim3(grid), dim3(512), 0, s, f); break;
    case 3: hipLaunchKernelGGL((lnb_fused16_kernel<KS, (KS + 1) / 2, 3>), dim3(grid), dim3(512), 0, s, f); break;
    default: hipLaunchKernelGGL((lnb_fused16_kernel<KS, (KS + 1) / 2, 0>), dim3(grid), dim3(512), 0, s, f);
  }
}
static int num_cus() {
  static int cache[64] = {};
  int dev = 0;
  if (hipGetDevice(&dev) != hipSuccess || dev < 0 || dev >= 64) return 256;
  if (!cache[dev]) {
    int n = 0;
    if (hipDeviceGetAttribute(&n, hipDeviceAttributeMultiprocessorCount, dev) != hipSuccess || n <= 0) n = 256;
    cache[dev] = n;
  }
  return cache[dev];
}

grr_status lnb_forward_mfma(const float* x, const float* ln_w, const float* w1, const float* wdw, const float* w2,
                            const float* skip, float* out, float* ws, int B, int C, int hid, int H, int W,
                            hipStream_t s, bool keep_g, int io) {
  GRR_REQUIRE(io == 0 || (lnb_fused(C, hid) && !keep_g), GRR_ERR_UNSUPPORTED,
              "grr_lnb_forward_c8: the channel-blocked layout needs the fused pass (C <= 96) without the kept gate");
  if (!lnb_fused(C, hid)) {
    return lnb_forward_mfma_rep(x, C, 1, x, ln_w, w1, wdw, w2, skip, out, ws, B, hid, H, W, s);
  }
  GRR_REQUIRE((int64_t)std::max(hid, C) * H * W * 4 < (1ll << 31), GRR_ERR_UNSUPPORTED,
              "grr_lnb_forward: max(hid, C)*H*W too large for one image's 32-bit offsets");
  const int KS = (C + 15) / 16, MT = (C + 31) / 32, nch = (hid + 15) / 16;
  const int64_t P = (int64_t)H * W;
  float* base = keep_g ? ws + align64((int64_t)B * hid * P) : ws;
  char* pack = reinterpret_cast<char*>(base);
  float* r2 = base + align64((int64_t)nch * fused_images(KS, MT) * 256);
  if (g_lnb_phases & 1) {
    const int64_t n = (int64_t)nch * fused_images(KS, MT) * 256 + C;
    hipLaunchKernelGGL(lnb_fused_pack_kernel, dim3((unsigned)std::min<int64_t>((n + 255) / 256, 4096)), dim3(256),
                       0, s, w1, ln_w, wdw, w2, pack, r2, C, hid, KS, MT, nch);
    grr_status st = launch_status("grr_lnb_forward/fused_pack");
    if (st != GRR_OK) return st;
  }
  if (!(g_lnb_phases & 2)) return GRR_OK;
  LnbFusedArgs f{};
  f.x = x; f.pack = pack; f.r2 = r2; f.skip = skip; f.out = out;
  f.g = keep_g ? ws : nullptr;
  f.var_den = (float)(C - 1);
  f.C = C; f.hid = hid; f.H = H; f.W = W; f.nch = nch;
  f.tiles_x = (W + LF_TW - 1) / LF_TW;
  f.tiles_y = (H + LF_TH - 1) / LF_TH;
  const uint64_t nt = (uint64_t)B * f.tiles_x * f.tiles_y;
  GRR_REQUIRE(nt < (1ull << 31), GRR_ERR_UNSUPPORTED, "grr_lnb_forward: grid too large");
  f.ntiles = (int)nt;
  const unsigned grid = (unsigned)std::min<uint64_t>(nt, (uint64_t)num_cus());
  switch (KS) {
    case 1: launch_fused<1>(f, grid, io, s); break;
    case 2: launch_fused<2>(f, grid, io, s); break;
    case 3: launch_fused<3>(f, grid, io, s); break;
    case 4: launch_fused<4>(f, grid, io, s); break;
    case 5: launch_fused<5>(f, grid, io, s); break;
    default: launch_fused<6>(f, grid, io, s); break;
  }
  return launch_status("grr_lnb_forward/fused");
}

bool lnb_rep_fused(int Ch, int R, int C, int hid) {
  return R > 1 && Ch >= 1 && Ch <= 3 && C <= 128 && hid >= 1;
}

template <int MT>
static void launch_rep(const LnbRepArgs& r, hipStream_t s) {
  switch (r.Cs) {
    case 1: hipLaunchKernelGGL((lnb_rep_kernel<MT, 1>), dim3(r.nblk), dim3(64 * LR_NW), 0, s, r); break;
    case 2: hipLaunchKernelGGL((lnb_rep_kernel<MT, 2>), dim3(r.nblk), dim3(64 * LR_NW), 0, s, r); break;
    default: hipLaunchKernelGGL((lnb_rep_kernel<MT, 3>), dim3(r.nblk), dim3(64 * LR_NW), 0, s, r); break;
  }
}

grr_status lnb_forward_mfma_rep(const float* xh, int Ch, int R, const float* x, const float* ln_w, const float* w1,
                                const float* wdw, const float* w2, const float* skip, float* out, float* ws, int B,
                                int hid, int H, int W, hipStream_t s) {
  const int C = R * Ch;
  GRR_REQUIRE(C >= 2 && C <= 128 && Ch >= 1, GRR_ERR_UNSUPPORTED, "grr_lnb_forward: C=%d outside [2, 128]", C);
  GRR_REQUIRE((int64_t)std::max(hid, C) * H * W * 4 < (1ll << 31), GRR_ERR_UNSUPPORTED,
              "grr_lnb_forward: max(hid, C)*H*W too large for one image's 32-bit offsets");
  if (lnb_rep_fused(Ch, R, C, hid)) {
    const int MT = (C + 31) / 32, nch = (hid + 15) / 16;
    char* pack = reinterpret_cast<char*>(ws);
    if (g_lnb_phases & 1) {
      const int64_t n = (int64_t)nch * rep_images(MT) * 256;
      hipLaunchKernelGGL(lnb_rep_pack_kernel, dim3((unsigned)std::min<int64_t>((n + 255) / 256, 4096)), dim3(256), 0,
                         s, w1, ln_w, wdw, w2, pack, Ch, R, C, hid, MT, nch);
      grr_status st = launch_status("grr_lnb_forward/rep_pack");
      if (st != GRR_OK) return st;
    }
    if (!(g_lnb_phases & 2)) return GRR_OK;
    LnbRepArgs r{};
    r.xs = xh; r.pack = pack; r.skip = skip; r.out = out;
    r.var_den = (float)(C - 1) / (float)R;
    r.Cs = Ch; r.C = C; r.hid = hid; r.H = H; r.W = W; r.nch = nch;
    r.tiles = (int)(((int64_t)H * W + LR_PX - 1) / LR_PX);
    const uint64_t nb = (uint64_t)B * r.tiles;
    GRR_REQUIRE(nb < (1ull << 31), GRR_ERR_UNSUPPORTED, "grr_lnb_forward: grid too large");
    r.nblk = (uint32_t)nb;
    switch (MT) {
      case 1: launch_rep<1>(r, s); break;
      case 2: launch_rep<2>(r, s); break;
      case 3: launch_rep<3>(r, s); break;
      default: launch_rep<4>(r, s); break;
    }
    return launch_status("grr_lnb_forward/rep");
  }
  const bool h16 = head16_enabled(Ch);
  const int KS = h16 ? head16_ks(Ch) : head_ks(Ch), NB = head_nb(head_ks(Ch));
  const int nch = h16 ? (hid + L6_NP - 1) / L6_NP : (hid + LH_JC - 1) / LH_JC;
  const int MT = (C + 31) / 32, KS2 = (hid + LM_KD - 1) / LM_KD;
  const int64_t P = (int64_t)H * W;
  float* g = ws;
  char* w1f = reinterpret_cast<char*>(ws + align64((int64_t)B * hid * P));
  uint16_t* w2f = reinterpret_cast<uint16_t*>(ws + align64((int64_t)B * hid * P) + head_pack_floats(Ch, hid));
  if (g_lnb_phases & 1) {
    const int64_t n1 = (int64_t)nch * (h16 ? head16_images(KS) : head_images(KS)) * 256;
    const int64_t n2 = (int64_t)KS2 * MT * 3 * 512;
    const dim3 g1((unsigned)std::min<int64_t>((n1 + 255) / 256, 4096));
    if (h16) hipLaunchKernelGGL(lnb_w1_pack16_kernel, g1, dim3(256), 0, s, w1, ln_w, wdw, w1f, Ch, hid, KS, nch, R);
    else hipLaunchKernelGGL(lnb_w1_pack_kernel, g1, dim3(256), 0, s, w1, ln_w, wdw, w1f, Ch, hid, KS, nch, R);
    hipLaunchKernelGGL(lnb_w2_pack_kernel, dim3((unsigned)std::min<int64_t>((n2 + 255) / 256, 4096)), dim3(256), 0,
                       s, w2, w2f, C, hid, MT, KS2);
    grr_status st = launch_status("grr_lnb_forward/pack");
    if (st != GRR_OK) return st;
  }
  LnbHeadArgs h{};
  h.x = xh; h.w1f = w1f; h.g = g;
  h.var_den = R == 1 ? (float)(C - 1) : (float)(C - 1) / (float)R;
  h.C = Ch; h.hid = hid; h.H = H; h.W = W; h.nch = nch;
  const int TH = h16 ? L6_TH : (NB == 4 ? HeadGeom<4>::TH : HeadGeom<3>::TH);
  h.tiles_x = (W + LH_TW - 1) / LH_TW;
  h.tiles_y = (H + TH - 1) / TH;
  const uint64_t nh = (uint64_t)B * h.tiles_x * h.tiles_y;
  GRR_REQUIRE(nh < (1ull << 31), GRR_ERR_UNSUPPORTED, "grr_lnb_forward: grid too large");
  h.nblk = (uint32_t)nh;
  if (!(g_lnb_phases & 2)) {
  } else if (h16) {
    switch (KS) {
      case 1: launch_head16<1>(h, s); break;
      case 2: launch_head16<2>(h, s); break;
      case 3: launch_head16<3>(h, s); break;
      case 4: launch_head16<4>(h, s); break;
      case 5: launch_head16<5>(h, s); break;
      default: launch_head16<6>(h, s); break;
    }
  } else {
    switch (KS) {
      case 1: launch_head<1, 4>(h, s); break;
      case 2: launch_head<2, 4>(h, s); break;
      case 3: launch_head<3, 4>(h, s); break;
      default: launch_head<4, 3>(h, s); break;
    }
  }
  grr_status st = launch_status("grr_lnb_forward/head");
  if (st != GRR_OK) return st;
  if (!(g_lnb_phases & 4)) return GRR_OK;
  LnbMixArgs m{};
  m.g = g; m.w2f = reinterpret_cast<const char*>(w2f); m.skip = skip; m.out = out;
  m.x = x ? x : xh;
  m.xs_c = x ? 0 : Ch;
  m.P = P; m.C = C; m.hid = hid; m.KS2 = KS2;
  m.tiles = (int)((P + LM_PX - 1) / LM_PX);
  const uint64_t nm = (uint64_t)B * m.tiles;
  GRR_REQUIRE(nm < (1ull << 31), GRR_ERR_UNSUPPORTED, "grr_lnb_forward: grid too large");
  m.nblk = (uint32_t)nm;
  const bool v4 = P % 4 == 0;
  switch (MT) {
    case 1: launch_mix<1>(m, v4, s); break;
    case 2: launch_mix<2>(m, v4, s); break;
    case 3: launch_mix<3>(m, v4, s); break;
    default: launch_mix<4>(m, v4, s); break;
  }
  return launch_status("grr_lnb_forward/mix");
}

}

extern "C" int grr_lnb_rep_fused(int Cs, int R, int C, int hid) { return grr::lnb_rep_fused(Cs, R, C, hid) ? 1 : 0; }
extern "C" int grr_lnb_fused(int C, int hid) { return grr::lnb_fused(C, hid) ? 1 : 0; }

extern "C" grr_status grr_lnb_set_fused(int enable) {
  grr::clear_error();
  GRR_REQUIRE(enable == 0 || enable == 1, GRR_ERR_INVALID_ARG, "grr_lnb_set_fused: 0 or 1");
  grr::g_lnb_fused_on = enable;
  return GRR_OK;
}

extern "C" grr_status grr_lnb_set_phases(int mask) {
  grr::clear_error();
  GRR_REQUIRE(mask >= 1 && mask <= 7, GRR_ERR_INVALID_ARG, "grr_lnb_set_phases: mask %d outside [1, 7]", mask);
// ... 5 lines not shown
```

imagerestoration-development-unrolling_amd/kernels.py:

```python
from __future__ import annotations

from typing import Optional, Sequence, Tuple

import os

import torch

from . import _native
from ._native import Stencil, call

Tensor = torch.Tensor


def _ptr(t: Optional[Tensor]):
    return None if t is None else t.data_ptr()


def _aligned16(t: Tensor) -> Tensor:
    return t if t.data_ptr() % 16 == 0 else t.clone()


def _check(name: str, *ts: Optional[Tensor]) -> torch.device:
    dev = None
    for t in ts:
        if t is None:
            continue
        if not t.is_cuda:
            raise RuntimeError(f"{name}: tensors must be on the GPU (got {t.device}); "
                               "the HIP engine has no CPU path")
        if t.dtype != torch.float32:
            raise TypeError(f"{name}: expected float32, got {t.dtype}")
        if not t.is_contiguous():
            raise ValueError(f"{name}: expected a contiguous tensor")
        if dev is None:
            dev = t.device
        elif t.device != dev:
            raise RuntimeError(f"{name}: tensors on different devices ({dev} vs {t.device})")
    return dev


def _stream(dev: torch.device):
    return torch.cuda.current_stream(dev).cuda_stream


class LaunchTimer:
    split_lnb = False

    def __init__(self):
        self.records = {}

    def run(self, kind: str, nbytes: int, fn, flops: int = 0):
        s = torch.cuda.Event(enable_timing=True)
        e = torch.cuda.Event(enable_timing=True)
        s.record()
        fn()
        e.record()
        self.records.setdefault(kind, []).append((s, e, nbytes, flops))

    def summary(self):
        torch.cuda.synchronize()
        out = {}
        for kind, recs in self.records.items():
            ms = [s.elapsed_time(e) for s, e, _, _ in recs]
            nb = sum(r[2] for r in recs)
            fl = sum(r[3] for r in recs)
            tot = sum(ms)
            out[kind] = {"launches": len(recs), "total_ms": tot, "mean_ms": tot / len(recs),
                         "bytes_per_launch": nb / len(recs), "gbps": nb / (tot * 1e-3) / 1e9 if tot > 0 else 0.0,
                         "flops_per_launch": fl / len(recs),
                         "tflops": fl / (tot * 1e-3) / 1e12 if tot > 0 else 0.0}
        return out


_TIMER = None


def set_timer(timer):
    global _TIMER
    _TIMER = timer


TIMER_SHAPES = os.environ.get("GRR_TIMER_SHAPES", "0") == "1"


def _launch(kind: str, nbytes: int, name: str, *args, flops: int = 0):
    if _TIMER is None:
        call(name, *args)
    else:
        _TIMER.run(kind, int(nbytes), lambda: call(name, *args), int(flops))


def lnb_flops(px: int, c_head: int, c: int, hid: int) -> int:
    return px * (4 * c_head + 2 * c_head * 2 * hid + 18 * 2 * hid + 4 * hid + 2 * hid * c + 3 * c)


def stencil(module) -> Stencil:
    ps = [module.stats_kernel_p01, module.stats_kernel_p02a, module.stats_kernel_p02b, module.stats_kernel_p03]
    _check("stencil", *[p.data for p in ps])
    return Stencil(*[p.data_ptr() for p in ps])


NO_STENCIL = Stencil(None, None, None, None)


TERM_ROWS = True


def set_term_rows(enable) -> None:
    global TERM_ROWS
    level = 2 if enable is True else int(enable)
    _native.call("grr_bwd_set_term_rows", level)
    TERM_ROWS = level > 0


def set_term_tail(enable: bool) -> None:
    _native.call("grr_bwd_set_term_tail", int(bool(enable)))


def set_term_acc_max_w(w: int) -> None:
    _native.call("grr_bwd_set_term_acc_max_w", int(w))


def term_rows_ok(w: int, f: int) -> bool:
    if w <= 64:
        return f <= 16
    if w <= 128 and w % 2 == 0:
        return f <= 16
    return w % 4 == 0 and f <= 12


def set_kernel_variant(variant: str) -> None:
    _native.call("grr_set_kernel_variant", {"auto": 0, "strips": 1, "independent": 2}[variant])


def stream_copy(src: Tensor, dst: Tensor) -> None:
    assert src.is_contiguous() and dst.is_contiguous() and src.numel() == dst.numel()
    call("grr_stream_copy", src.data_ptr(), dst.data_ptr(), src.numel(), _stream(src.device))


def neighbor_table(h: int, w: int, device) -> Tensor:
    out = torch.empty((4, h, w), dtype=torch.int32, device=device)
    call("grr_neighbor_table", out.data_ptr(), h, w, _stream(out.device))
    return out


def edge_weights(feat: Tensor, channel_offset: int, n_graphs: int, n_fts: int, multiM: Tensor,
                 with_degree: bool = False) -> Tuple[Tensor, Optional[Tensor]]:
    dev = _check("edge_weights", feat, multiM)
    b, ctot, h, w = feat.shape
    if channel_offset + n_graphs * n_fts > ctot:
        raise ValueError("edge_weights: channel slab out of range")
    wt = torch.empty((b, n_graphs, 4, h, w), dtype=torch.float32, device=dev)
    deg = torch.empty((b, n_graphs, h, w), dtype=torch.float32, device=dev) if with_degree else None
    base = feat.data_ptr() + channel_offset * h * w * feat.element_size()
    nbytes = 4 * b * h * w * (n_graphs * n_fts + 4 * n_graphs + (n_graphs if with_degree else 0))
    _launch("edge_weights", nbytes, "grr_edge_weights", base, ctot * h * w, multiM.data_ptr(), wt.data_ptr(),
            _ptr(deg), b, n_graphs, n_fts, h, w, _stream(dev))
# ... 417 lines not shown
def conv1x1_cat2_ok(ka: int, kb: int, m: int, p: int) -> bool:
    k = ka + kb
    return (ka >= 16 and ka % 16 == 0 and kb >= 1 and k <= 4096 and 1 <= m <= (1 << 20) and p >= 1
            and (k + 16) * p < (1 << 30) and (m + 128) * p < (1 << 30))


def _embed_shapes(name: str, x: Tensor, weight: Tensor) -> Tuple[int, int, int, int, int]:
    if x.dim() != 4 or weight.dim() != 4:
        raise ValueError(f"{name}: expected x [B,Cin,H,W] and weight [M,Cin,3,3]")
    b, cin, h, w = x.shape
    m = weight.shape[0]
    if tuple(weight.shape[1:]) != (cin, 3, 3):
        raise ValueError(f"{name}: weight {tuple(weight.shape)} vs input channels {cin}")
    if not conv3x3_embed_ok(cin, m) or min(b, h, w) < 1:
        raise ValueError(f"{name}: Cin={cin}, M={m} outside the kernel's range (Cin <= 4, M <= 128)")
    return b, cin, m, h, w


def conv3x3_embed(x: Tensor, weight: Tensor) -> Tensor:
    dev = _check("conv3x3_embed", x, weight)
    b, cin, m, h, w = _embed_shapes("conv3x3_embed", x, weight)
    out = torch.empty((b, m, h, w), dtype=torch.float32, device=dev)
    _launch("conv3x3_embed", 4 * b * h * w * (cin + m), "grr_conv3x3_embed", x.data_ptr(), weight.data_ptr(),
            out.data_ptr(), b, cin, m, h, w, _stream(dev), flops=2 * b * h * w * 9 * cin * m)
    return out


def conv3x3_embed_bwd_w(g: Tensor, x: Tensor) -> Tensor:
    dev = _check("conv3x3_embed_bwd_w", g, x)
    if x.dim() != 4 or g.dim() != 4 or g.shape[0] != x.shape[0] or g.shape[2:] != x.shape[2:]:
        raise ValueError(f"conv3x3_embed_bwd_w: g {tuple(g.shape)} vs x {tuple(x.shape)}")
    b, cin, h, w = x.shape
    m = g.shape[1]
    if not conv3x3_embed_ok(cin, m) or min(b, h, w) < 1:
        raise ValueError(f"conv3x3_embed_bwd_w: Cin={cin}, M={m} outside the kernel's range (Cin <= 4, M <= 128)")
    g = _aligned16(g)
    gw = torch.empty((m, cin, 3, 3), dtype=torch.float32, device=dev)
    ws = _ws(_native.load().grr_conv3x3_embed_bwd_w_workspace_bytes(b, cin, m, h, w), dev)
    _launch("conv3x3_embed_bwd_w", 4 * b * h * w * (m + cin + 18 * cin), "grr_conv3x3_embed_bwd_w", g.data_ptr(),
            x.data_ptr(), gw.data_ptr(), ws.data_ptr(), b, cin, m, h, w, _stream(dev),
            flops=2 * b * h * w * 9 * cin * m)
    return gw


def conv3x3_embed_bwd_x(g: Tensor, weight: Tensor) -> Tensor:
    dev = _check("conv3x3_embed_bwd_x", g, weight)
    if g.dim() != 4 or weight.dim() != 4 or tuple(weight.shape[2:]) != (3, 3) or weight.shape[0] != g.shape[1]:
        raise ValueError(f"conv3x3_embed_bwd_x: g {tuple(g.shape)} vs weight {tuple(weight.shape)}")
    b, m, h, w = g.shape
    cin = weight.shape[1]
    if not conv3x3_embed_ok(cin, m) or min(b, h, w) < 1:
        raise ValueError(f"conv3x3_embed_bwd_x: Cin={cin}, M={m} outside the kernel's range (Cin <= 4, M <= 128)")
    gx = torch.empty((b, cin, h, w), dtype=torch.float32, device=dev)
    _launch("conv3x3_embed_bwd_x", 4 * b * h * w * (m + cin), "grr_conv3x3_embed_bwd_x", g.data_ptr(),
            weight.data_ptr(), gx.data_ptr(), b, cin, m, h, w, _stream(dev), flops=2 * b * h * w * 9 * cin * m)
    return gx


def convt2x2s2(x: Tensor, weight: Tensor) -> Tensor:
    dev = _check("convt2x2s2", x, weight)
    if x.dim() != 4 or weight.dim() != 4:
        raise ValueError("convt2x2s2: expected x [B,K,H,W] and weight [K,M,2,2]")
    b, k, h, w = x.shape
    m = weight.shape[1]
    if tuple(weight.shape) != (k, m, 2, 2):
        raise ValueError(f"convt2x2s2: weight {tuple(weight.shape)} vs input channels {k}")
    if not convt2x2s2_ok(k, m, h, w) or b < 1:
        raise ValueError(f"convt2x2s2: shape {tuple(x.shape)} -> {m} channels outside the kernel's range")
    out = torch.empty((b, m, 2 * h, 2 * w), dtype=torch.float32, device=dev)
    ws = _ws(_native.load().grr_convt2x2s2_workspace_bytes(b, k, m, h, w), dev)
    kind = f"convt2x2s2[{k}->{m},{b}x{h}x{w}]" if TIMER_SHAPES else "convt2x2s2"
    _launch(kind, 4 * b * h * w * (k + 4 * m), "grr_convt2x2s2", x.data_ptr(), weight.data_ptr(), out.data_ptr(),
            ws.data_ptr(), b, k, m, h, w, _stream(dev), flops=2 * b * h * w * k * 4 * m)
    return out


def conv1x1_cat2(xa: Tensor, xb: Tensor, weight: Tensor) -> Tensor:
    dev = _check("conv1x1_cat2", xa, xb, weight)
    if xa.dim() != 4 or xb.dim() != 4 or xa.shape[0] != xb.shape[0] or xa.shape[2:] != xb.shape[2:]:
        raise ValueError(f"conv1x1_cat2: inputs {tuple(xa.shape)} and {tuple(xb.shape)} disagree")
    b, ka, h, w = xa.shape
    kb = xb.shape[1]
    m = weight.shape[0]
    if weight.numel() != m * (ka + kb) or weight.shape[1] != ka + kb:
        raise ValueError(f"conv1x1_cat2: weight {tuple(weight.shape)} vs input channels {ka} + {kb}")
    if not conv1x1_cat2_ok(ka, kb, m, h * w):
        return conv1x1(torch.cat([xa, xb], 1), weight)
    out = torch.empty((b, m, h, w), dtype=torch.float32, device=dev)
    ws = _ws(_native.load().grr_conv1x1_cat2_workspace_bytes(ka, kb, m), dev)
    kind = f"conv1x1_cat2[{ka}+{kb}->{m},{b}x{h}x{w}]" if TIMER_SHAPES else "conv1x1_cat2"
    _launch(kind, 4 * b * h * w * (ka + kb + m), "grr_conv1x1_cat2", xa.data_ptr(), xb.data_ptr(), weight.data_ptr(),
            out.data_ptr(), ws.data_ptr(), b, ka, kb, m, h * w, _stream(dev), flops=2 * b * h * w * (ka + kb) * m)
    return out


def ffn_forward(x: Tensor, ln_w: Tensor, w_in: Tensor, w_dw: Tensor, w_out: Tensor, skip: Tensor) -> Tensor:
    dev = _check("ffn_forward", x, ln_w, w_in, w_dw, w_out, skip)
    b, c, h, w = x.shape
    hid = w_out.shape[1]
    if tuple(w_in.shape) != (2 * hid, c) or tuple(w_dw.shape) != (2 * hid, 9) or tuple(w_out.shape) != (c, hid) \
            or ln_w.numel() != c or skip.numel() != 2:
        raise ValueError("ffn_forward: weight shapes disagree with x / hid")
    out = torch.empty_like(x)
    ws = torch.empty((_native.load().grr_ffn_workspace_bytes(b, c, hid, h, w) + 3) // 4, dtype=torch.float32,
                     device=dev)
    p = b * h * w
    _launch("ffn", 4 * p * (2 * c + 3 * hid + 2 * hid), "grr_ffn_forward", x.data_ptr(), ln_w.data_ptr(),
            w_in.data_ptr(), w_dw.data_ptr(), w_out.data_ptr(), skip.data_ptr(), out.data_ptr(), ws.data_ptr(),
            b, c, hid, h, w, _stream(dev), flops=p * (2 * c * 2 * hid + 18 * 2 * hid + 2 * hid * c))
    return out


def wgrad(a: Tensor, bop: Tensor) -> Tensor:
    dev = _check("wgrad", a, bop)
    a, bop = _aligned16(a), _aligned16(bop)
    b, m = a.shape[:2]
    k = bop.shape[1]
    p = a.numel() // (b * m)
    if bop.shape[0] != b or bop.numel() != b * k * p:
        raise ValueError(f"wgrad: operands {tuple(a.shape)} and {tuple(bop.shape)} disagree")
    out = torch.empty((m, k), dtype=torch.float32, device=dev)
    ws = torch.empty((_native.load().grr_wgrad_workspace_bytes(b, m, k, p) + 3) // 4, dtype=torch.float32,
                     device=dev)
    _launch(f"wgrad[{m}x{k},{b}x{p}]" if TIMER_SHAPES else "wgrad", 4 * b * p * (m + k), "grr_wgrad", a.data_ptr(), bop.data_ptr(), out.data_ptr(), ws.data_ptr(),
            b, m, k, p, _stream(dev), flops=2 * b * p * m * k)
    return out


def set_wgrad_tiles(enable: bool) -> None:
    _native.call("grr_wgrad_set_tiles", int(bool(enable)))


_WS_CACHE = {}


_LNB_MAX_BYTES = 1 << 31


def _lnb_band_rows(c: int, hid: int, h: int, w: int) -> int:
    per_row = max(hid, c) * w * 4
    return h if per_row * h < _LNB_MAX_BYTES else max(1, (_LNB_MAX_BYTES - 1) // per_row - 2)


def _lnb_banded(run, xs, h: int, rows: int) -> Tensor:
    outs = []
    for r0 in range(0, h, rows):
        r1 = min(r0 + rows, h)
        a, e = max(r0 - 1, 0), min(r1 + 1, h)
        y = run(*[None if t is None else t[:, :, a:e].contiguous() for t in xs])
        outs.append(y[:, :, r0 - a:r1 - a])
    return torch.cat(outs, 2)


def lnb_forward(x: Tensor, ln_w: Tensor, w1: Tensor, wdw: Tensor, w2: Tensor, skip: Tensor) -> Tensor:
    dev = _check("lnb_forward", x, ln_w, w1, wdw, w2, skip)
    b, c, h, w = x.shape
    hid = w2.shape[1]
    rows = _lnb_band_rows(c, hid, h, w)
    if rows < h:
        return _lnb_banded(lambda xb: lnb_forward(xb, ln_w, w1, wdw, w2, skip), [x], h, rows)
    lib = _native.load()
    fused = bool(lib.grr_lnb_fused(c, hid))
    nbytes = lib.grr_lnb_fused_workspace_bytes(c, hid) if fused else lib.grr_lnb_workspace_bytes(b, c, hid, h, w)
    ws = torch.empty((nbytes + 3) // 4, dtype=torch.float32, device=dev)
    out = torch.empty_like(x)
    args = (x.data_ptr(), ln_w.data_ptr(), w1.data_ptr(), wdw.data_ptr(), w2.data_ptr(), skip.data_ptr(),
            out.data_ptr(), ws.data_ptr(), b, c, hid, h, w, _stream(dev))
    if fused:
        _launch("lnb_fused", 4 * b * h * w * 2 * c, "grr_lnb_forward", *args, flops=lnb_flops(b * h * w, c, c, hid))
        return out
    if _lnb_split(c):
        _lnb_timed_parts("grr_lnb_forward", args, b * h * w, c, c, hid, c)
        return out
    nbytes_algo = 4 * b * h * w * (3 * c + 2 * hid) if c <= 128 else 4 * b * h * w * (3 * c + 2 * (2 * hid) + 2 * hid)
    _launch("lnb", nbytes_algo, "grr_lnb_forward", *args, flops=lnb_flops(b * h * w, c, c, hid))
    return out


def c8_shape(b: int, c: int, h: int, w: int) -> Tuple[int, int, int, int, int]:
    return (b, (c + 7) // 8, h, w, 8)


def to_c8(x: Tensor) -> Tensor:
    dev = _check("to_c8", x)
    b, c, h, w = x.shape
    y = torch.empty(c8_shape(b, c, h, w), dtype=torch.float32, device=dev)
    _launch("c8_convert", 8 * y.numel(), "grr_c8_convert", x.contiguous().data_ptr(), y.data_ptr(), b, c, h, w, 1,
            _stream(dev))
    return y


def from_c8(y: Tensor, c: int) -> Tensor:
    dev = _check("from_c8", y)
    b, nb, h, w, _ = y.shape
    x = torch.empty((b, c, h, w), dtype=torch.float32, device=dev)
    _launch("c8_convert", 8 * x.numel(), "grr_c8_convert", y.data_ptr(), x.data_ptr(), b, c, h, w, 0, _stream(dev))
    return x


LNB_FUSED = True


def set_lnb_fused(enable: bool) -> None:
    global LNB_FUSED
    _native.call("grr_lnb_set_fused", int(bool(enable)))
    LNB_FUSED = bool(enable)


def lnb_c8_ok(c: int, hid: int, h: int, w: int) -> bool:
    return LNB_FUSED and 2 <= c <= 96 and hid >= 1 and _lnb_band_rows(c, hid, h, w) >= h and \
        ((c + 7) // 8) * 8 * h * w * 4 < (1 << 31)


def lnb_forward_c8(x: Tensor, c: int, ln_w: Tensor, w1: Tensor, wdw: Tensor, w2: Tensor, skip: Tensor,
                   in_c8: bool, out_c8: bool) -> Tensor:
    dev = _check("lnb_forward_c8", x, ln_w, w1, wdw, w2, skip)
    if in_c8:
        b, _, h, w, _ = x.shape
    else:
        b, c_in, h, w = x.shape
        if c_in != c:
            raise ValueError("lnb_forward_c8: channels")
    hid = w2.shape[1]
    lib = _native.load()
    ws = torch.empty((lib.grr_lnb_fused_workspace_bytes(c, hid) + 3) // 4, dtype=torch.float32, device=dev)
    out = torch.empty(c8_shape(b, c, h, w) if out_c8 else (b, c, h, w), dtype=torch.float32, device=dev)
    xc = x.contiguous()
    _launch("lnb_fused", 4 * b * h * w * 2 * c, "grr_lnb_forward_c8", xc.data_ptr(), ln_w.data_ptr(), w1.data_ptr(),
            wdw.data_ptr(), w2.data_ptr(), skip.data_ptr(), out.data_ptr(), ws.data_ptr(), b, c, hid, h, w,
            int(in_c8) | 2 * int(out_c8), _stream(dev), flops=lnb_flops(b * h * w, c, c, hid))
    return out


def lnb_gate_keepable(c: int, hid: int, h: int, w: int) -> bool:
    return 2 <= c <= 128 and _lnb_band_rows(c, hid, h, w) >= h


def lnb_forward_keep(x: Tensor, ln_w: Tensor, w1: Tensor, wdw: Tensor, w2: Tensor,
                     skip: Tensor) -> Tuple[Tensor, Tensor]:
    dev = _check("lnb_forward_keep", x, ln_w, w1, wdw, w2, skip)
    b, c, h, w = x.shape
    hid = w2.shape[1]
    if not lnb_gate_keepable(c, hid, h, w):
        raise ValueError("lnb_forward_keep: needs C <= 128 and one band")
    nbytes = _native.load().grr_lnb_workspace_bytes(b, c, hid, h, w)
    ws = torch.empty((nbytes + 3) // 4, dtype=torch.float32, device=dev)
    out = torch.empty_like(x)
    args = (x.data_ptr(), ln_w.data_ptr(), w1.data_ptr(), wdw.data_ptr(), w2.data_ptr(), skip.data_ptr(),
            out.data_ptr(), ws.data_ptr(), b, c, hid, h, w, _stream(dev))
    if _native.load().grr_lnb_fused(c, hid):
        _launch("lnb_fused", 4 * b * h * w * (2 * c + hid), "grr_lnb_forward_keep", *args,
                flops=lnb_flops(b * h * w, c, c, hid))
    elif _lnb_split(c):
        _lnb_timed_parts("grr_lnb_forward_keep", args, b * h * w, c, c, hid, c)
    else:
        _launch("lnb", 4 * b * h * w * (3 * c + 2 * hid), "grr_lnb_forward_keep", *args,
                flops=lnb_flops(b * h * w, c, c, hid))
    return out, ws[:b * hid * h * w].view(b, hid, h, w)


def lnb_forward_rep(src: Tensor, x: Optional[Tensor], ln_w: Tensor, w1: Tensor, wdw: Tensor, w2: Tensor,
                    skip: Tensor) -> Tensor:
    dev = _check("lnb_forward_rep", src, x, ln_w, w1, wdw, w2, skip)
    b, cs, h, w = src.shape
    c = ln_w.numel()
    if c % cs or (x is not None and tuple(x.shape) != (b, c, h, w)):
        raise ValueError("lnb_forward_rep: the block input must be copies of src")
    hid = w2.shape[1]
    rows = _lnb_band_rows(c, hid, h, w)
    if rows < h:
        return _lnb_banded(lambda sb, xb: lnb_forward_rep(sb, xb, ln_w, w1, wdw, w2, skip), [src, x], h, rows)
    nbytes = _native.load().grr_lnb_workspace_bytes(b, c, hid, h, w)
    ws = torch.empty((nbytes + 3) // 4, dtype=torch.float32, device=dev)
    out = torch.empty((b, c, h, w), dtype=torch.float32, device=dev)
    args = (src.data_ptr(), cs, c // cs, _ptr(x), ln_w.data_ptr(), w1.data_ptr(), wdw.data_ptr(), w2.data_ptr(),
            skip.data_ptr(), out.data_ptr(), ws.data_ptr(), b, hid, h, w, _stream(dev))
    if _native.load().grr_lnb_rep_fused(cs, c // cs, c, hid):
        _launch("lnb_rep_fused", 4 * b * h * w * (cs + 2 * c if x is not None else cs + c), "grr_lnb_forward_rep",
                *args, flops=lnb_flops(b * h * w, cs, c, hid))
        return out
    if _lnb_split(c):
        _lnb_timed_parts("grr_lnb_forward_rep", args, b * h * w, cs, c, hid, c if x is not None else cs)
        return out
    _launch("lnb", 4 * b * h * w * (cs + 2 * c + 2 * hid), "grr_lnb_forward_rep", *args,
            flops=lnb_flops(b * h * w, cs, c, hid))
    return out


def _lnb_split(c: int) -> bool:
    return _TIMER is not None and getattr(_TIMER, "split_lnb", False) and c <= 128


def lnb_head_flops(px: int, c_head: int, hid: int) -> int:
    return px * (4 * c_head + 2 * c_head * 2 * hid + 18 * 2 * hid + 4 * hid)


def _lnb_timed_parts(name: str, args, px: int, c_head: int, c: int, hid: int, c_skip: int) -> None:
    try:
        call("grr_lnb_set_phases", 3)
        _launch("lnb_head", 4 * px * (c_head + hid), name, *args, flops=lnb_head_flops(px, c_head, hid))
        call("grr_lnb_set_phases", 4)
        _launch("lnb_mix", 4 * px * (hid + c_skip + c), name, *args, flops=px * (2 * hid * c + 3 * c))
    finally:
        call("grr_lnb_set_phases", 7)


def repeat_graphs(img: Tensor, n_graphs: int) -> Tensor:
    dev = _check("repeat_graphs", img)
    b, cin, h, w = img.shape
    out = torch.empty((b, n_graphs * cin, h, w), dtype=torch.float32, device=dev)
    _launch("repeat_graphs", 4 * b * h * w * cin * (1 + n_graphs), "grr_repeat_graphs", img.data_ptr(),
            out.data_ptr(), b, cin, n_graphs, h * w, _stream(dev))
    return out


ST_P, ST_T, ST_T_ADJ, ST_P_ADJ = 0, 1, 2, 3


def stencil_taps(p01: Tensor, p02a: Tensor, p02b: Tensor, p03: Tensor) -> Tensor:
    a, b, c, d = (t.reshape(-1) for t in (p01, p02a, p02b, p03))
    return torch.stack([a - b - c + 4 * d, -d, -d, b - d, c - d], dim=1).contiguous()


def stencil_taps_backward(gt: Tensor):
    dc, du, dl, dr, dd = gt.unbind(1)
    out = (dc, dr - dc, dd - dc, 4 * dc - du - dl - dr - dd)
    return tuple(t.reshape(-1, 1, 1, 1) for t in out)


def _bgfhw(x: Tensor, n_graphs: int):
    b, c, h, w = x.shape
    if c % n_graphs:
        raise ValueError(f"{c} channels not divisible by {n_graphs} graphs")
    return b, n_graphs, c // n_graphs, h, w


def bwd_stencil(x: Tensor, taps: Tensor, mode: int, n_graphs: int, scale: Optional[Tensor] = None,
                out: Optional[Tensor] = None) -> Tensor:
    dev = _check("bwd_stencil", x, taps, scale, out)
    acc = out is not None
    if out is None:
        out = torch.empty_like(x)
    _launch("bwd_stencil", 4 * x.numel() * (3 if acc else 2), "grr_bwd_stencil", x.data_ptr(), taps.data_ptr(), mode,
            _ptr(scale), int(acc), out.data_ptr(), *_bgfhw(x, n_graphs), _stream(dev))
    return out


def padj2_ok(x: Tensor) -> bool:
    return x.shape[3] % 4 == 0


def bwd_padj2(v1: Tensor, taps1: Tensor, scale1: Tensor, v2: Tensor, taps2: Tensor, scale2: Tensor, out: Tensor,
              n_graphs: int) -> None:
    dev = _check("bwd_padj2", v1, taps1, scale1, v2, taps2, scale2, out)
    _launch("bwd_stencil", 4 * v1.numel() * 4, "grr_bwd_padj2", v1.data_ptr(), taps1.data_ptr(), scale1.data_ptr(),
            v2.data_ptr(), taps2.data_ptr(), scale2.data_ptr(), out.data_ptr(), *_bgfhw(v1, n_graphs), _stream(dev))


def bwd_tapgrad(u: Tensor, z: Tensor, mode: int, n_graphs: int, scale: Optional[Tensor], gtaps: Tensor) -> None:
    dev = _check("bwd_tapgrad", u, z, scale, gtaps)
    _launch("bwd_tapgrad", 8 * u.numel(), "grr_bwd_tapgrad", u.data_ptr(), z.data_ptr(), mode, _ptr(scale),
            gtaps.data_ptr(), *_bgfhw(u, n_graphs), _stream(dev))


def bwd_glr(s: Tensor, a: Tensor, w: Tensor, scale: Tensor, coef: float, gw: Tensor, gdot: Tensor, n_graphs: int):
    dev = _check("bwd_glr", s, a, w, scale, gw, gdot)
    z, ap = torch.empty_like(s), torch.empty_like(s)
    _launch("bwd_glr", 4 * (4 * s.numel() + 3 * w.numel()), "grr_bwd_glr", s.data_ptr(), a.data_ptr(), w.data_ptr(),
            scale.data_ptr(), float(coef), z.data_ptr(), ap.data_ptr(), gw.data_ptr(), _ptr(gdot),
            *_bgfhw(s, n_graphs), _stream(dev))
    return z, ap


def bwd_pair(s: Tensor, a: Tensor, c: Tensor, scale: Tensor, coef: float, gc: Tensor, gdot: Tensor, n_graphs: int):
    dev = _check("bwd_pair", s, a, c, scale, gc, gdot)
    z, ap = torch.empty_like(s), torch.empty_like(s)
    _launch("bwd_pair", 4 * (4 * s.numel() + 3 * c.numel()), "grr_bwd_pair", s.data_ptr(), a.data_ptr(), c.data_ptr(),
            scale.data_ptr(), float(coef), z.data_ptr(), ap.data_ptr(), gc.data_ptr(), _ptr(gdot),
            *_bgfhw(s, n_graphs), _stream(dev))
    return z, ap
# ... 629 lines not shown
```

include/grr.h:

```cpp
#ifndef GRR_H
#define GRR_H

#include <stdint.h>

#ifdef __cplusplus
extern "C" {
#endif

typedef enum grr_status {
  GRR_OK = 0,
  GRR_ERR_INVALID_ARG = 1,
  GRR_ERR_SHAPE = 2,
  GRR_ERR_UNSUPPORTED = 3,
  GRR_ERR_HIP = 4
} grr_status;

#define GRR_MAX_NODE_FTS 24

int grr_version(void);
const char* grr_last_error(void);

grr_status grr_set_kernel_variant(int variant);
grr_status grr_lnb_set_phases(int mask);

// ... 17 lines not shown
                                  int B, int G, int F, int H, int W, void* stream);

grr_status grr_pool2(const float* x, float* xd, int B, int C, int H, int W, void* stream);

typedef struct grr_stencil {
  const float* p01;
  const float* p02a;
  const float* p02b;
  const float* p03;
} grr_stencil;

grr_status grr_system_half(const float* xd, const float* wL, const float* cG,
                           grr_stencil sL, grr_stencil sG,
                           const float* log_mu, const float* log_ro,
                           float* t, int B, int G, int F, int h, int w, void* stream);

grr_status grr_gtv_rhs_half(const float* xd, const float* wG, grr_stencil sG, int prox,
                            const float* log_gamma, float* t,
                            int B, int G, int F, int h, int w, void* stream);

grr_status grr_gtv_rhs_full(const float* x, const float* y, const float* wG, grr_stencil sG,
                            int prox, const float* log_gamma, const float* log_ro0,
                            const float* t_half, const float* log_ro1,
                            float* b_out, float* xd_out,
                            int B, int G, int F, int H, int W, void* stream);

grr_status grr_gtv_rhs_full_rep(const float* x, int x_rep, const float* y, int y_rep, const float* wG,
                                grr_stencil sG, int prox, const float* log_gamma, const float* log_ro0,
                                const float* t_half, const float* log_ro1, float* b_out, float* xd_out,
                                int B, int G, int F, int H, int W, void* stream);

grr_status grr_system_step(const float* x, const float* b, const float* u_prev, const float* t_half,
                           const float* wL, const float* cG, grr_stencil sL, grr_stencil sG,
                           const float* log_mu0, const float* log_ro0,
                           const float* alpha, const float* beta,
                           const float* skip, const float* y_skip,
                           float* x_out, float* u_out, float* xd_out,
                           int B, int G, int F, int H, int W, void* stream);

grr_status grr_system_step2(const float* x, const float* b, const float* u_prev, const float* xd,
                            const float* wL0, const float* cG0, grr_stencil sL0, grr_stencil sG0,
                            const float* log_mu0, const float* log_ro0, const float* wL1, const float* cG1,
                            grr_stencil sL1, grr_stencil sG1, const float* log_mu1, const float* log_ro1,
                            const float* alpha_a, const float* beta_a, const float* alpha_b, const float* beta_b,
                            const float* skip, const float* y_skip, float* x_out, float* u_out, float* xd_out,
                            int B, int G, int F, int H, int W, void* stream);
grr_status grr_system_first_pair(const float* b_a, const float* xd_a, const float* y, int y_rep, const float* wL0,
                                 const float* cG0, const float* wG0, grr_stencil sL0, grr_stencil sG0,
                                 const float* log_mu0, const float* log_ro0, const float* log_gamma0,
                                 const float* wL1, const float* cG1, const float* wG1, grr_stencil sL1,
                                 grr_stencil sG1, const float* log_mu1, const float* log_ro1,
                                 const float* log_gamma1, const float* alpha0, const float* alpha1, float* b_out,
                                 float* x_out, float* u_out, float* xd_out, int B, int G, int F, int H, int W,
                                 void* stream);
grr_status grr_system_step2_train(const float* x, const float* b, const float* u_prev, const float* xd,
                                  const float* wL0, const float* cG0, grr_stencil sL0, grr_stencil sG0,
                                  const float* log_mu0, const float* log_ro0, const float* wL1, const float* cG1,
                                  grr_stencil sL1, grr_stencil sG1, const float* log_mu1, const float* log_ro1,
                                  const float* alpha_a, const float* beta_a, const float* alpha_b,
                                  const float* beta_b, float* x_out, float* u_out, float* xd_out, float* x_mid,
                                  float* u_mid, float* xd_mid, int B, int G, int F, int H, int W, void* stream);

grr_status grr_glr_stage(const float* x, const float* b, const float* u_prev, const float* wL, grr_stencil sL,
                         const float* mu, const float* alpha, const float* beta, float* x_out, float* u_out,
                         int B, int G, int F, int H, int W, void* stream);


grr_status grr_neighbor_gather(const float* x, float* out, int B, int C, int H, int W, void* stream);
grr_status grr_normalize_features(const float* f, const float* multiM, float* out, int B, int G, int F, int H, int W,
                                  void* stream);
grr_status grr_stats_conv(const float* x, grr_stencil s, int transpose, float* out, int B, int G, int F, int H, int W,
                          void* stream);
grr_status grr_glr_op_l_norm(const float* x, const float* w, float* out, int B, int G, int F, int H, int W,
                             void* stream);
grr_status grr_gtv_op_c(const float* x, const float* w, grr_stencil s, float* edges, int B, int G, int F, int H, int W,
                        void* stream);
grr_status grr_gtv_op_c_transpose(const float* edges, const float* w, grr_stencil s, float* work, float* out, int B,
                                  int G, int F, int H, int W, void* stream);

grr_status grr_neighbor_gather_bwd(const float* g, float* gx, int B, int C, int H, int W, void* stream);
grr_status grr_normalize_features_bwd(const float* f, const float* multiM, const float* gout, float* gf, float* gM,
                                      int B, int G, int F, int H, int W, void* stream);
grr_status grr_stats_conv_bwd(const float* x, grr_stencil s, int transpose, const float* g, float* gx, float* gtaps,
                              int B, int G, int F, int H, int W, void* stream);
grr_status grr_glr_op_l_norm_bwd(const float* x, const float* w, const float* g, float* gx, float* gw, int B, int G,
                                 int F, int H, int W, void* stream);
grr_status grr_gtv_op_c_bwd(const float* x, const float* w, grr_stencil s, const float* gE, float* work, float* gx,
                            float* gw, float* gtaps, int B, int G, int F, int H, int W, void* stream);
grr_status grr_gtv_op_c_transpose_bwd(const float* edges, const float* w, grr_stencil s, const float* z,
                                      const float* g, float* work2, float* gE, float* gw, float* gtaps, int B, int G,
                                      int F, int H, int W, void* stream);


grr_status grr_conv1x1(const float* x, const float* wt, float* out, int B, int K, int M, int64_t P,
                       void* stream);

int64_t grr_conv1x1_workspace_bytes(int K, int M);
grr_status grr_conv1x1_ws(const float* x, const float* wt, float* out, void* workspace, int B, int K, int M,
                          int64_t P, void* stream);

grr_status grr_conv2x2s2(const float* x, const float* wt, float* out, int B, int K, int M, int H, int W,
                         void* stream);


int grr_conv3x3_embed_supported(int Cin, int M);
grr_status grr_conv3x3_embed(const float* x, const float* wt, float* out, int B, int Cin, int M, int H, int W,
                             void* stream);
int64_t grr_conv3x3_embed_bwd_w_workspace_bytes(int B, int Cin, int M, int H, int W);
grr_status grr_conv3x3_embed_bwd_w(const float* g, const float* x, float* gw, void* workspace, int B, int Cin, int M,
                                   int H, int W, void* stream);
grr_status grr_conv3x3_embed_bwd_x(const float* g, const float* wt, float* gx, int B, int Cin, int M, int H, int W,
                                   void* stream);

int64_t grr_convt2x2s2_workspace_bytes(int B, int K, int M, int H, int W);
grr_status grr_convt2x2s2(const float* x, const float* wt, float* out, void* workspace, int B, int K, int M, int H,
                          int W, void* stream);

int grr_conv1x1_cat2_supported(int Ka, int Kb, int M, int64_t P);
int64_t grr_conv1x1_cat2_workspace_bytes(int Ka, int Kb, int M);
grr_status grr_conv1x1_cat2(const float* xa, const float* xb, const float* wt, float* out, void* workspace, int B,
                            int Ka, int Kb, int M, int64_t P, void* stream);

int64_t grr_ffn_workspace_bytes(int B, int C, int hid, int H, int W);
grr_status grr_ffn_forward(const float* x, const float* ln_w, const float* w_in, const float* w_dw, const float* w_out,
                           const float* skip, float* out, void* workspace, int B, int C, int hid, int H, int W,
                           void* stream);

int64_t grr_wgrad_workspace_bytes(int B, int M, int K, int64_t P);
grr_status grr_wgrad_set_tiles(int enable);
grr_status grr_wgrad(const float* a, const float* bop, float* out, void* workspace, int B, int M, int K, int64_t P,
                     void* stream);

int64_t grr_lnb_workspace_bytes(int B, int C, int hid, int H, int W);
grr_status grr_lnb_forward(const float* x, const float* ln_w, const float* w1, const float* wdw,
                           const float* w2, const float* skip, float* out, void* workspace,
                           int B, int C, int hid, int H, int W, void* stream);

int grr_feature_edges_supported(int C, int G, int F, int H, int W);
int64_t grr_feature_edges_workspace_bytes(int G);
grr_status grr_feature_edges(const float* x, int x_blocked, const float* wf, const float* multiM_gtv,
                             const float* multiM_glr, float* wG, float* cG, float* wL, void* workspace, int B,
                             int C, int G, int F, int H, int W, void* stream);

grr_status grr_lnb_forward_c8(const float* x, const float* ln_w, const float* w1, const float* wdw,
                              const float* w2, const float* skip, float* out, void* workspace, int B, int C,
                              int hid, int H, int W, int layout, void* stream);
grr_status grr_c8_convert(const float* src, float* dst, int B, int C, int H, int W, int to_blocked, void* stream);

grr_status grr_lnb_forward_keep(const float* x, const float* ln_w, const float* w1, const float* wdw,
                                const float* w2, const float* skip, float* out, void* workspace, int B, int C,
                                int hid, int H, int W, void* stream);
int grr_lnb_fused(int C, int hid);
int64_t grr_lnb_fused_workspace_bytes(int C, int hid);
grr_status grr_lnb_set_fused(int enable);
grr_status grr_lnb_forward_rep(const float* src, int Cs, int R, const float* x, const float* ln_w, const float* w1,
                               const float* wdw, const float* w2, const float* skip, float* out, void* workspace,
                               int B, int hid, int H, int W, void* stream);
int grr_lnb_rep_fused(int Cs, int R, int C, int hid);

grr_status grr_repeat_graphs(const float* img, float* out, int B, int Cin, int G, int64_t P, void* stream);


grr_status grr_bwd_stencil(const float* x, const float* taps, int mode, const float* scale, int accumulate,
                           float* out, int B, int G, int F, int H, int W, void* stream);
grr_status grr_bwd_padj2(const float* v1, const float* taps1, const float* scale1, const float* v2, const float* taps2,
                         const float* scale2, float* out, int B, int G, int F, int H, int W, void* stream);
grr_status grr_bwd_tapgrad(const float* u, const float* z, int mode, const float* scale, float* gtaps,
                           int B, int G, int F, int H, int W, void* stream);
grr_status grr_bwd_glr(const float* s, const float* a, const float* w, const float* scale, float coef,
                       float* z_out, float* ap_out, float* gw, float* gdot,
                       int B, int G, int F, int H, int W, void* stream);
grr_status grr_bwd_pair(const float* s, const float* a, const float* c, const float* scale, float coef,
                        float* z_out, float* ap_out, float* gc, float* gdot,
                        int B, int G, int F, int H, int W, void* stream);
grr_status grr_bwd_prox(const float* s, const float* a, const float* w, const float* log_gamma,
                        const float* scale, float coef, float* o_out, float* gs_out, float* gw,
                        float* ggamma, float* gdot, int B, int G, int F, int H, int W, void* stream);
grr_status grr_bwd_set_term_acc_max_w(int w);
grr_status grr_bwd_set_term_rows(int enable);
grr_status grr_bwd_set_term_tail(int enable);

grr_status grr_bwd_term_fused(int mode, const float* x, const float* g, const float* taps, const float* w,
                              const float* log_gamma, const float* scale, float coef, float* v_out, float* gw,
                              float* ggamma, float* gdot, float* gtaps, int B, int G, int F, int H, int W,
                              void* stream);
int grr_bwd_term_acc_supported(int mode, int F, int H, int W);
grr_status grr_bwd_term_fused_acc(int mode, const float* x, const float* g, const float* taps, const float* w,
                                  const float* log_gamma, const float* scale, float coef, float* gx, float* gw,
                                  float* ggamma, float* gdot, float* gtaps, int B, int G, int F, int H, int W,
                                  void* stream);
grr_status grr_bwd_pair_weights(const float* w, const float* gc, float* gw, int B, int G, int H, int W,
                                void* stream);
grr_status grr_bwd_edge_weights(const float* feat, int64_t feat_bstride, const float* multiM, const float* w,
                                const float* gw, float* gfeat, int64_t gfeat_bstride, float* gmultiM,
                                int B, int G, int F, int H, int W, void* stream);
grr_status grr_bwd_graph_dot(const float* u, const float* v, float coef, float* gdot,
                             int B, int G, int F, int H, int W, void* stream);
grr_status grr_bwd_cg_glue(const float* gx, const float* gx_half, const float* v1, const float* taps1,
                           const float* scale1, const float* v2, const float* taps2, const float* scale2,
                           const float* u, const float* gu_next, const float* u_prev, const float* alpha,
                           const float* beta_next, float* gu, float* gbb, float* gx_out, float* galpha, float* gbeta,
                           int B, int G, int F, int H, int W, void* stream);
grr_status grr_bwd_cg_glue_pool(const float* gx, const float* gx_half, const float* v1, const float* taps1,
                                const float* scale1, const float* v2, const float* taps2, const float* scale2,
                                const float* u, const float* gu_next, const float* u_prev, const float* alpha,
                                const float* beta_next, float* gu, float* gbb, float* gx_out, float* gu_half,
                                float* galpha, float* gbeta, int B, int G, int F, int H, int W, void* stream);
grr_status grr_bwd_lincomb(const float* x, const float* sa, const float* y, const float* sb, float* out,
                           int accumulate, int B, int G, int F, int H, int W, void* stream);
grr_status grr_bwd_unpool2_acc(const float* xd, float* out, int B, int C, int H, int W, void* stream);
grr_status grr_interleave2x2(const float* t, float* gx, int B, int K, int H, int W, void* stream);
grr_status grr_conv2x2s2_bwd_data(const float* g, const float* wt, float* gx, int B, int K, int M, int H, int W,
                                  void* stream);

grr_status grr_lnb_norm(const float* x, const float* ln_w, float* n, float* isd, int B, int C, int64_t P,
                        void* stream);
grr_status grr_lnb_norm_bwd(const float* x, const float* ln_w, const float* isd, const float* gn, float* gx,
                            float* gln_w, int B, int C, int64_t P, void* stream);
grr_status grr_lnb_norm_bwd_skip(const float* x, const float* ln_w, const float* isd, const float* gn,
                                 const float* gout, const float* skip, float* gx, float* gln_w, float* gskip0, int B,
                                 int C, int64_t P, void* stream);
grr_status grr_dwconv3(const float* h, const float* wdw, float* out, int B, int C, int H, int W, void* stream);
grr_status grr_dwconv3_bwd(const float* g, const float* h, const float* wdw, float* gh, float* gwdw, int B, int C,
                           int H, int W, void* stream);
grr_status grr_lnb_gate(const float* hp, const float* ggate, float* gate, float* ghp, int B, int hid, int64_t P,
                        void* stream);
grr_status grr_lnb_gate_bwd_scaled(const float* hp, const float* gq, const float* scale, float* ghp, float* gdot, int B,
                                   int hid, int64_t P, void* stream);
grr_status grr_lnb_dw3_gate(const float* hh, const float* wdw, float* gate, int B, int hid, int H, int W,
                            void* stream);
grr_status grr_lnb_set_bwd_ring(int enable);
grr_status grr_dw3_ring_check(int W);
grr_status grr_lnb_gate_dw3_bwd(const float* hp, const float* gq, const float* scale, const float* hh,
                                const float* wdw, float* gh, float* gwdw, float* gdot, int B, int hid, int H, int W,
                                void* stream);

grr_status grr_ffn_dw3_gate(const float* hh, const float* wdw, float* gate, int B, int hid, int H, int W,
                            void* stream);
grr_status grr_ffn_gate_dw3_bwd(const float* gq, const float* scale, const float* hh, const float* wdw, float* gh,
                                float* gwdw, float* gdot, int B, int hid, int H, int W, void* stream);


grr_status grr_win_edge_weights(const float* feat, int64_t feat_bstride, const float* multiM, const int32_t* delta,
                                int K, float* w, float* deg, int B, int G, int F, int H, int W, void* stream);

grr_status grr_win_solver(int mode, const float* x, int x_rep, const float* y, const float* u_prev, const float* wL,
                          const float* wG, const float* tapsL, const float* tapsG, const float* mu, const float* ro,
                          const float* log_gamma, const float* alpha, const float* beta, const int32_t* delta, int K,
                          float* out, float* u_out, int B, int G, int Fs, int H, int W, void* stream);

grr_status grr_win_pair_weights(const float* w, const int32_t* delta, int K, float* c, int B, int G, int H, int W,
                                void* stream);

grr_status grr_win_mix(const float* x, const float* score, const float* dc, float* out, int B, int G, int Fs, int H,
                       int W, void* stream);


grr_status grr_win_bwd_stencil(const float* x, const float* taps, int mode, const float* scale, int accumulate,
                               float* out, int B, int G, int Fs, int H, int W, void* stream);
grr_status grr_win_bwd_tapgrad(const float* u, const float* z, int mode, const float* scale, float* gtaps, int B,
                               int G, int Fs, int H, int W, void* stream);
grr_status grr_win_bwd_glr(const float* s, const float* b, const float* w, const int32_t* delta, int K,
                           const float* scale, float coef, float* l_out, float* E, float* gsd, float* gw, float* gdot,
                           int B, int G, int Fs, int H, int W, void* stream);
grr_status grr_win_bwd_gtv(const float* s, const float* b, const float* w, const int32_t* delta, int K, int prox,
                           const float* log_gamma, const float* scale, float coef, float* PW, float* E, float* gsd,
                           float* gw, float* gdot, float* ggamma, int B, int G, int Fs, int H, int W, void* stream);
grr_status grr_win_bwd_gather(const float* E, const float* PW, const int32_t* delta, int K, float* gs, float* o_out,
                              int B, int G, int Fs, int H, int W, void* stream);
grr_status grr_win_bwd_gather_fused(const float* s, const float* b, const float* w, const int32_t* delta, int K,
                                    int gtv, int prox, const float* log_gamma, const float* scale, float* gs,
                                    float* o_out, int B, int G, int Fs, int H, int W, void* stream);
grr_status grr_win_bwd_edge_weights(const float* feat, int64_t feat_bstride, const float* multiM, const float* w,
                                    float* gw, const int32_t* delta, int K, float* gfeat, int64_t gfeat_bstride,
                                    float* gmultiM, int B, int G, int F, int H, int W, void* stream);
grr_status grr_win_bwd_mix(const float* gout, const float* x, const float* score, float* gx, float* gscore, int B,
                           int G, int Fs, int H, int W, void* stream);


int grr_image_io_supported(int C, int H, int W);
grr_status grr_tile_gather(const void* img, int img_f32, int H, int W, int C, const int32_t* table, int n, int th,
                           int tw, float* out, void* stream);
grr_status grr_tile_scatter(const float* y, const int32_t* table, int n, int th, int tw, void* img, int img_f32, int H,
                            int W, int C, void* stream);
grr_status grr_u8_sse(const uint8_t* a, const uint8_t* b, int64_t n, uint64_t* out, void* stream);

#ifdef __cplusplus
}
#endif

#endif
```

Before: 148.1 MPix/s.

## Cache packed LNB weights and spread fused GEMM work across all eight waves

```diff
diff --git a/imagerestoration-development-unrolling_amd/_native.py b/imagerestoration-development-unrolling_amd/_native.py
--- a/imagerestoration-development-unrolling_amd/_native.py
+++ b/imagerestoration-development-unrolling_amd/_native.py
@@ -81,6 +81,8 @@
     "grr_lnb_forward": [P, P, P, P, P, P, P, P, I, I, I, I, I, P],
     "grr_lnb_forward_keep": [P, P, P, P, P, P, P, P, I, I, I, I, I, P],
     "grr_lnb_forward_c8": [P, P, P, P, P, P, P, P, I, I, I, I, I, I, P],
+    "grr_lnb_fused_pack": [P, P, P, P, P, I, I, P],
+    "grr_lnb_forward_packed": [P, P, P, P, I, I, I, I, I, I, P],
     "grr_c8_convert": [P, P, I, I, I, I, I, P],
     "grr_feature_edges_supported": [I, I, I, I, I],
     "grr_feature_edges_workspace_bytes": [I],
diff --git a/imagerestoration-development-unrolling_amd/csrc/feature_ops.hip b/imagerestoration-development-unrolling_amd/csrc/feature_ops.hip
--- a/imagerestoration-development-unrolling_amd/csrc/feature_ops.hip
+++ b/imagerestoration-development-unrolling_amd/csrc/feature_ops.hip
@@ -942,6 +942,31 @@
                                (hipStream_t)stream, false, layout);
 }
 
+grr_status grr_lnb_fused_pack(const float* ln_w, const float* w1, const float* wdw, const float* w2, void* packed,
+                              int C, int hid, void* stream) {
+  grr::clear_error();
+  GRR_REQUIRE(ln_w && w1 && wdw && w2 && packed && C > 1 && hid > 0, GRR_ERR_INVALID_ARG, "grr_lnb_fused_pack: bad args");
+  GRR_REQUIRE(((uintptr_t)packed & 255) == 0, GRR_ERR_INVALID_ARG, "grr_lnb_fused_pack: packed not 256-B aligned");
+  GRR_REQUIRE(grr_lnb_fused(C, hid), GRR_ERR_UNSUPPORTED, "grr_lnb_fused_pack: needs the fused pass (grr_lnb_fused)");
+  return grr::lnb_forward_mfma(nullptr, ln_w, w1, wdw, w2, nullptr, nullptr, (float*)packed, 1, C, hid, 1, 1,
+                               (hipStream_t)stream, false, 0, 1);
+}
+
+grr_status grr_lnb_forward_packed(const float* x, const void* packed, const float* skip, float* out, int B, int C,
+                                  int hid, int H, int W, int layout, void* stream) {
+  grr::clear_error();
+  GRR_REQUIRE(x && packed && skip && out && B > 0 && C > 1 && hid > 0 && H > 0 && W > 0 && layout >= 0 && layout <= 3,
+              GRR_ERR_INVALID_ARG, "grr_lnb_forward_packed: bad args");
+  GRR_REQUIRE(out != x, GRR_ERR_INVALID_ARG, "grr_lnb_forward_packed: out aliases x");
+  GRR_REQUIRE(((uintptr_t)packed & 255) == 0 && (layout == 0 || (((uintptr_t)x & 15) == 0 && ((uintptr_t)out & 15) == 0)),
+              GRR_ERR_INVALID_ARG, "grr_lnb_forward_packed: packed 256-B, blocked x and out 16-B aligned");
+  GRR_REQUIRE(grr_lnb_fused(C, hid) && (int64_t)((C + 7) / 8) * 8 * H * W * 4 < (1ll << 31), GRR_ERR_UNSUPPORTED,
+              "grr_lnb_forward_packed: needs the fused pass (grr_lnb_fused) and 2^31 bytes per blocked image");
+  return grr::lnb_forward_mfma(x, nullptr, nullptr, nullptr, nullptr, skip, out,
+                               const_cast<float*>(static_cast<const float*>(packed)), B, C, hid, H, W,
+                               (hipStream_t)stream, false, layout, 2);
+}
+
 namespace grr {
 __global__ __launch_bounds__(256) void c8_pack_kernel(const float* __restrict__ x, float* __restrict__ y, int C, int64_t HW,
                                                      int64_t n) {
diff --git a/imagerestoration-development-unrolling_amd/csrc/grr_common.h b/imagerestoration-development-unrolling_amd/csrc/grr_common.h
--- a/imagerestoration-development-unrolling_amd/csrc/grr_common.h
+++ b/imagerestoration-development-unrolling_amd/csrc/grr_common.h
@@ -38,7 +38,7 @@
 bool lnb_fused(int C, int hid);
 grr_status lnb_forward_mfma(const float* x, const float* ln_w, const float* w1, const float* wdw, const float* w2,
                             const float* skip, float* out, float* ws, int B, int C, int hid, int H, int W,
-                            hipStream_t s, bool keep_g = false, int io = 0);
+                            hipStream_t s, bool keep_g = false, int io = 0, int parts = 3);
 grr_status lnb_forward_mfma_rep(const float* xh, int Ch, int R, const float* x, const float* ln_w, const float* w1,
                                 const float* wdw, const float* w2, const float* skip, float* out, float* ws, int B,
                                 int hid, int H, int W, hipStream_t s);
diff --git a/imagerestoration-development-unrolling_amd/csrc/lnb_ops.hip b/imagerestoration-development-unrolling_amd/csrc/lnb_ops.hip
--- a/imagerestoration-development-unrolling_amd/csrc/lnb_ops.hip
+++ b/imagerestoration-development-unrolling_amd/csrc/lnb_ops.hip
@@ -948,8 +948,29 @@
 #ifndef GRR_FUSED_STAMP
 #define GRR_FUSED_STAMP 0
 #endif
+#ifndef GRR_FUSED_PKFMA
+#define GRR_FUSED_PKFMA 0
+#endif
+#ifndef GRR_FUSED_EARLYX
+#define GRR_FUSED_EARLYX 1
+#endif
+__device__ __forceinline__ f32x4 lf_mul4(const f32x4& t, const f32x4& w) {
+#if GRR_FUSED_PKFMA
+  return t * w;
+#else
+  return f32x4{t[0] * w[0], t[1] * w[1], t[2] * w[2], t[3] * w[3]};
+#endif
+}
+__device__ __forceinline__ f32x4 lf_fma4(const f32x4& t, const f32x4& w, const f32x4& s) {
+#if GRR_FUSED_PKFMA
+  return __builtin_elementwise_fma(t, w, s);
+#else
+  return f32x4{__builtin_fmaf(t[0], w[0], s[0]), __builtin_fmaf(t[1], w[1], s[1]), __builtin_fmaf(t[2], w[2], s[2]),
+               __builtin_fmaf(t[3], w[3], s[3])};
+#endif
+}
 #if GRR_FUSED_STAMP
-__device__ unsigned long long g_fused_stamps[1024 * 8 * 8];
+__device__ unsigned long long g_fused_stamps[512 * 8 * 16];
 #define FSTAMP(k)                                              \
   do {                                                         \
     const unsigned long long t_ = __builtin_amdgcn_s_memtime(); \
@@ -1006,13 +1027,13 @@
   };
   if (nsteps == 0) return;
 #if GRR_FUSED_STAMP
-  unsigned long long st_acc[8] = {}, st_prev = __builtin_amdgcn_s_memtime();
+  unsigned long long st_acc[9] = {}, st_prev = __builtin_amdgcn_s_memtime();
   auto stamp_out = [&]() {
-    if (lane < 8 && blockIdx.x < 1024) {
+    if (lane < 9 && blockIdx.x < 512) {
       unsigned long long v = 0;
 #pragma unroll
-      for (int k = 0; k < 8; ++k) v = lane == k ? st_acc[k] : v;
-      g_fused_stamps[(blockIdx.x * 8 + wave) * 8 + lane] = v;
+      for (int k = 0; k < 9; ++k) v = lane == k ? st_acc[k] : v;
+      g_fused_stamps[(blockIdx.x * 8 + wave) * 16 + lane] = v;
     }
   };
 #endif
@@ -1021,280 +1042,273 @@
   __builtin_amdgcn_s_barrier();
   asm volatile("" ::: "memory");
 
-  if (wave < 4) {
-    constexpr int NBW = (LF_NBLK + 3) / 4;
-    const bool has_last = wave + 4 * (NBW - 1) < LF_NBLK;
-    f16x8 xh[NBW][KS], xl[NBW][KS];
-    float corr[NBW];
-    bool wave_corr = false;
-    int c = 0, tile = wg, sl = 0;
-    for (int i = 0; i <= nsteps; ++i) {
+  constexpr int NBW = (LF_NBLK + 7) / 8;
+  const bool has_last = wave + 8 * (NBW - 1) < LF_NBLK;
+  const bool g1_first = wave < 4;
+  const int col = lane & 31;
+  f16x8 xh[NBW][KS], xl[NBW][KS];
+  float corr[NBW];
+  bool wave_corr = false, x_raw = false;
+  int c = 0, tile = wg, sl = 0;
+  f32x16 acc2[MT];
+  int E = 1000;
+  int ch = 0, ctile = wg, csl = 0;
+  FusedTile T2 = fused_tile(a, wg);
+
+  auto load_x = [&]() __attribute__((always_inline)) {
+    const FusedTile T = fused_tile(a, tile);
+    const int cx = IN8 ? 8 * ((C + 7) / 8) : C;
+    const __amdgpu_buffer_rsrc_t xr = __builtin_amdgcn_make_buffer_rsrc(
+        const_cast<float*>(a.x + (int64_t)T.b * cx * HW), 0, (int)((int64_t)cx * HW * 4), 0x00020000);
+#pragma unroll
+    for (int k = 0; k < NBW; ++k) {
+      if (k == NBW - 1 && !has_last) continue;
+      const int q = min((wave + 8 * k) * 32 + (lane & 31), LF_NQ - 1);
+      const int hy = q / LF_HWD, hx = q - hy * LF_HWD;
+      const int gy = clampi(T.y0 - 1 + hy, 0, H - 1), gx = clampi(T.x0 - 1 + hx, 0, W - 1);
+      const int vo = (8 * kh * HW + gy * W + gx) * 4;
+      int hw4 = HW * 4;
+      asm volatile("" : "+s"(hw4));
+      if constexpr (IN8) {
+        const uint32_t vo8 = (uint32_t)((kh * HW + gy * W + gx) * 32);
+#pragma unroll
+        for (int s = 0; s < KS; ++s) {
+          xh[k][s] = __builtin_bit_cast(f16x8, __builtin_amdgcn_raw_buffer_load_b128(xr, vo8, 16 * s * hw4, 0));
+          xl[k][s] = __builtin_bit_cast(f16x8, __builtin_amdgcn_raw_buffer_load_b128(xr, vo8 + 16, 16 * s * hw4, 0));
+        }
+      } else {
+#pragma unroll
+        for (int s = 0; s < KS; ++s) {
+          u32x4 lo, hi;
+#pragma unroll
+          for (int j = 0; j < 4; ++j) {
+            lo[j] = __builtin_amdgcn_raw_buffer_load_b32(xr, vo, (16 * s + j) * hw4, 0);
+            hi[j] = __builtin_amdgcn_raw_buffer_load_b32(xr, vo, (16 * s + 4 + j) * hw4, 0);
+          }
+          xh[k][s] = __builtin_bit_cast(f16x8, lo);
+          xl[k][s] = __builtin_bit_cast(f16x8, hi);
+        }
+      }
+    }
+    x_raw = true;
+  };
+  auto convert_x = [&]() __attribute__((always_inline)) {
+    bool any_corr = false;
+#pragma unroll
+    for (int k = 0; k < NBW; ++k) {
+      if (k == NBW - 1 && !has_last) continue;
+      float xv[KS][8];
+#pragma unroll
+      for (int s = 0; s < KS; ++s) {
+        const u32x4 lo = __builtin_bit_cast(u32x4, xh[k][s]), hi = __builtin_bit_cast(u32x4, xl[k][s]);
+#pragma unroll
+        for (int j = 0; j < 4; ++j) {
+          xv[s][j] = __uint_as_float(lo[j]);
+          xv[s][4 + j] = __uint_as_float(hi[j]);
+        }
+      }
+      float sum = 0.f;
+#pragma unroll
+      for (int s = 0; s < KS; ++s)
+#pragma unroll
+        for (int j = 0; j < 8; ++j) sum += xv[s][j];
+      sum += __shfl_xor(sum, 32);
+      const float mean = sum / (float)C;
+      float sq = 0.f;
+#pragma unroll
+      for (int s = 0; s < KS; ++s)
+#pragma unroll
+        for (int j = 0; j < 8; ++j) {
+          const float d = 16 * s + 8 * kh + j < C ? xv[s][j] - mean : 0.f;
+          sq += d * d;
+        }
+      sq += __shfl_xor(sq, 32);
+      const float rstd = 1.0f / sqrtf(sq / a.var_den + 1e-5f);
+      float mx = 0.f;
+#pragma unroll
+      for (int s = 0; s < KS; ++s)
+#pragma unroll
+        for (int j = 0; j < 8; ++j) {
+          xv[s][j] *= rstd;
+          mx = fmaxf(mx, fabsf(xv[s][j]));
+        }
+      mx = fmaxf(mx, __shfl_xor(mx, 32));
+      int ep = LF_XE;
+      if (mx != 0.f) {
+        int e;
+        frexpf(mx, &e);
+        if (e > 14 - LF_XE || e < -LF_XE) ep = clampi(14 - e, -100, 100);
+      }
+      corr[k] = ldexpf(1.0f, LF_XE - ep);
+      any_corr |= ep != LF_XE;
+#pragma unroll
+      for (int s = 0; s < KS; ++s) {
+        uint32_t hw[4], lw[4];
+#pragma unroll
+        for (int j = 0; j < 4; ++j)
+          split2_f16(ldexpf(xv[s][2 * j], ep), ldexpf(xv[s][2 * j + 1], ep), hw[j], lw[j]);
+        xh[k][s] = __builtin_bit_cast(f16x8, u32x4{hw[0], hw[1], hw[2], hw[3]});
+        xl[k][s] = __builtin_bit_cast(f16x8, u32x4{lw[0], lw[1], lw[2], lw[3]});
+      }
+    }
+    wave_corr = __builtin_amdgcn_readfirstlane((int)__any(any_corr)) != 0;
+    x_raw = false;
+  };
+
+  if (GRR_FUSED_EARLYX) load_x();
+  auto sync_step = [&](int i) __attribute__((always_inline)) {
+    asm volatile("s_waitcnt vmcnt(0) lgkmcnt(0)" ::: "memory");
+    FSTAMP(7);
+    __builtin_amdgcn_s_barrier();
+    asm volatile("" ::: "memory");
+    FSTAMP(8);
+    if (i < nsteps) {
       issue(dsl, dch);
       advance_dma();
-      FSTAMP(0);
-      if (i < nsteps && !(GRR_FUSED_DIAG & 2)) {
-        if (c == 0) {
-          const FusedTile T = fused_tile(a, tile);
-          const int cx = IN8 ? 8 * ((C + 7) / 8) : C;
-          const __amdgpu_buffer_rsrc_t xr = __builtin_amdgcn_make_buffer_rsrc(
-              const_cast<float*>(a.x + (int64_t)T.b * cx * HW), 0, (int)((int64_t)cx * HW * 4), 0x00020000);
-          bool any_corr = false;
-#pragma unroll
-          for (int k = 0; k < NBW; ++k) {
-            const int q = min((wave + 4 * k) * 32 + (lane & 31), LF_NQ - 1);
-            const int hy = q / LF_HWD, hx = q - hy * LF_HWD;
-            const int gy = clampi(T.y0 - 1 + hy, 0, H - 1), gx = clampi(T.x0 - 1 + hx, 0, W - 1);
-            const int vo = (8 * kh * HW + gy * W + gx) * 4;
-            int hw4 = HW * 4;
-            asm volatile("" : "+s"(hw4));
-            float xv[KS][8];
-            if constexpr (IN8) {
-              const uint32_t vo8 = (uint32_t)((kh * HW + gy * W + gx) * 32);
-#pragma unroll
-              for (int s = 0; s < KS; ++s) {
-                const u32x4 lo = __builtin_bit_cast(u32x4, __builtin_amdgcn_raw_buffer_load_b128(xr, vo8, 16 * s * hw4, 0));
-                const u32x4 hi = __builtin_bit_cast(u32x4, __builtin_amdgcn_raw_buffer_load_b128(xr, vo8 + 16, 16 * s * hw4, 0));
-#pragma unroll
-                for (int j = 0; j < 4; ++j) {
-                  xv[s][j] = __uint_as_float(lo[j]);
-                  xv[s][4 + j] = __uint_as_float(hi[j]);
-                }
-              }
-            } else {
-#pragma unroll
-              for (int s = 0; s < KS; ++s)
-#pragma unroll
-                for (int j = 0; j < 8; ++j)
-                  xv[s][j] = __uint_as_float(__builtin_amdgcn_raw_buffer_load_b32(xr, vo, (16 * s + j) * hw4, 0));
-            }
-            float sum = 0.f;
-#pragma unroll
-            for (int s = 0; s < KS; ++s)
-#pragma unroll
-              for (int j = 0; j < 8; ++j) sum += xv[s][j];
-            sum += __shfl_xor(sum, 32);
-            const float mean = sum / (float)C;
-            float sq = 0.f;
-#pragma unroll
-            for (int s = 0; s < KS; ++s)
-#pragma unroll
-              for (int j = 0; j < 8; ++j) {
-                const float d = 16 * s + 8 * kh + j < C ? xv[s][j] - mean : 0.f;
-                sq += d * d;
-              }
-            sq += __shfl_xor(sq, 32);
-            const float rstd = 1.0f / sqrtf(sq / a.var_den + 1e-5f);
-            float mx = 0.f;
-#pragma unroll
-            for (int s = 0; s < KS; ++s)
-#pragma unroll
-              for (int j = 0; j < 8; ++j) {
-                xv[s][j] *= rstd;
-                mx = fmaxf(mx, fabsf(xv[s][j]));
-              }
-            mx = fmaxf(mx, __shfl_xor(mx, 32));
-            int ep = LF_XE;
-            if (mx != 0.f) {
-              int e;
-              frexpf(mx, &e);
-              if (e > 14 - LF_XE || e < -LF_XE) ep = clampi(14 - e, -100, 100);
-            }
-            corr[k] = ldexpf(1.0f, LF_XE - ep);
-            any_corr |= ep != LF_XE;
-#pragma unroll
-            for (int s = 0; s < KS; ++s) {
-              uint32_t hw[4], lw[4];
-#pragma unroll
-              for (int j = 0; j < 4; ++j)
-                split2_f16(ldexpf(xv[s][2 * j], ep), ldexpf(xv[s][2 * j + 1], ep), hw[j], lw[j]);
-              xh[k][s] = __builtin_bit_cast(f16x8, u32x4{hw[0], hw[1], hw[2], hw[3]});
-              xl[k][s] = __builtin_bit_cast(f16x8, u32x4{lw[0], lw[1], lw[2], lw[3]});
-            }
-          }
-          wave_corr = __builtin_amdgcn_readfirstlane((int)__any(any_corr)) != 0;
-        }
-        FSTAMP(1);
-        const float* slot = ring + sl * SLOTF + lane * 4;
-        f32x16 acc[NBW];
-#pragma unroll
-        for (int k = 0; k < NBW; ++k) acc[k] = f32x16{};
-        f16x8 ah = *reinterpret_cast<const f16x8*>(slot);
-        f16x8 al = *reinterpret_cast<const f16x8*>(slot + 256);
-#pragma unroll
-        for (int s = 0; s < KS; ++s) {
-          f16x8 bh, bl;
-          if (s + 1 < KS) {
-            bh = *reinterpret_cast<const f16x8*>(slot + (2 * s + 2) * 256);
-            bl = *reinterpret_cast<const f16x8*>(slot + (2 * s + 3) * 256);
-          }
-#pragma unroll
-          for (int k = 0; k < NBW; ++k) {
-            if (k == NBW - 1 && !has_last) continue;
-            acc[k] = __builtin_amdgcn_mfma_f32_32x32x16_f16(al, xh[k][s], acc[k], 0, 0, 0);
-            acc[k] = __builtin_amdgcn_mfma_f32_32x32x16_f16(ah, xl[k][s], acc[k], 0, 0, 0);
-            acc[k] = __builtin_amdgcn_mfma_f32_32x32x16_f16(ah, xh[k][s], acc[k], 0, 0, 0);
-          }
-          if (s + 1 < KS) {
-            ah = bh;
-            al = bl;
-          }
-          __builtin_amdgcn_sched_barrier(0);
-        }
-        FSTAMP(2);
-        float* hb = smem + (i & 1) * LF_HBUF;
+    }
+    FSTAMP(0);
+  };
+  issue(dsl, dch);
+  advance_dma();
+  FSTAMP(0);
+  for (int i = 0; i <= nsteps; ++i) {
+    if (i < nsteps && !(GRR_FUSED_DIAG & 2)) {
+      if (c == 0) {
+        if (!x_raw) load_x();
+        convert_x();
+      }
+      FSTAMP(1);
+      const float* slot = ring + sl * SLOTF + lane * 4;
+      f32x16 acc[NBW];
+#pragma unroll
+      for (int k = 0; k < NBW; ++k) acc[k] = f32x16{};
+      f16x8 ah = *reinterpret_cast<const f16x8*>(slot);
+      f16x8 al = *reinterpret_cast<const f16x8*>(slot + 256);
+#pragma unroll
+      for (int s = 0; s < KS; ++s) {
+        f16x8 bh, bl;
+        if (s + 1 < KS) {
+          bh = *reinterpret_cast<const f16x8*>(slot + (2 * s + 2) * 256);
+          bl = *reinterpret_cast<const f16x8*>(slot + (2 * s + 3) * 256);
+        }
 #pragma unroll
         for (int k = 0; k < NBW; ++k) {
           if (k == NBW - 1 && !has_last) continue;
-          if (wave_corr) acc[k] *= corr[k];
-          const int q = (wave + 4 * k) * 32 + (lane & 31);
-#pragma unroll
-          for (int u = 0; u < 4; ++u)
-            *reinterpret_cast<f32x4*>(hb + (2 * u + kh) * 2 * LF_PP + 4 * q) =
-                f32x4{acc[k][4 * u], acc[k][4 * u + 1], acc[k][4 * u + 2], acc[k][4 * u + 3]};
-        }
-        if (++c == nch) {
-          c = 0;
-          tile += G;
-        }
-        sl = sl == LF_NSLOT - 1 ? 0 : sl + 1;
-      }
+          acc[k] = __builtin_amdgcn_mfma_f32_32x32x16_f16(al, xh[k][s], acc[k], 0, 0, 0);
+          acc[k] = __builtin_amdgcn_mfma_f32_32x32x16_f16(ah, xl[k][s], acc[k], 0, 0, 0);
+          acc[k] = __builtin_amdgcn_mfma_f32_32x32x16_f16(ah, xh[k][s], acc[k], 0, 0, 0);
+        }
+        if (s + 1 < KS) {
+          ah = bh;
+          al = bl;
+        }
+        __builtin_amdgcn_sched_barrier(0);
+      }
+      FSTAMP(2);
+      float* hb = smem + (i & 1) * LF_HBUF;
+#pragma unroll
+      for (int k = 0; k < NBW; ++k) {
+        if (k == NBW - 1 && !has_last) continue;
+        if (wave_corr) acc[k] *= corr[k];
+        const int q = (wave + 8 * k) * 32 + (lane & 31);
+#pragma unroll
+        for (int u = 0; u < 4; ++u)
+          *reinterpret_cast<f32x4*>(hb + (2 * u + kh) * 2 * LF_PP + 4 * q) =
+              f32x4{acc[k][4 * u], acc[k][4 * u + 1], acc[k][4 * u + 2], acc[k][4 * u + 3]};
+      }
+      if (++c == nch) {
+        c = 0;
+        tile += G;
+      }
+      sl = sl == LF_NSLOT - 1 ? 0 : sl + 1;
       FSTAMP(3);
-      asm volatile("s_waitcnt vmcnt(0) lgkmcnt(0)" ::: "memory");
-      FSTAMP(4);
-      __builtin_amdgcn_s_barrier();
-      asm volatile("" ::: "memory");
-      FSTAMP(5);
-    }
-#if GRR_FUSED_STAMP
-    stamp_out();
-#endif
-    return;
-  }
-
-  __builtin_amdgcn_s_setprio(1);
-  const int cw = wave - 4;
-  const int col = lane & 31;
-  f32x16 acc2[2][MT];
-  int E[2] = {1000, 1000};
-  int ch = 0, ctile = wg, csl = 0;
-  for (int i = 0; i <= nsteps; ++i) {
-    issue(dsl, dch);
-    advance_dma();
-    FSTAMP(0);
-    if (i >= 1 && !(GRR_FUSED_DIAG & 1)) {
-      const int st = i - 1;
+    }
+    if (!g1_first) sync_step(i);
+    if (GRR_FUSED_EARLYX && c == 0 && !x_raw && tile < a.ntiles && !(GRR_FUSED_DIAG & 2)) load_x();
+    FSTAMP(1);
+    const int st = g1_first ? i - 1 : i;
+    if (st >= 0 && st < nsteps && !(GRR_FUSED_DIAG & 1)) {
+      __builtin_amdgcn_s_setprio(1);
       if (ch == 0) {
 #pragma unroll
-        for (int rb = 0; rb < 2; ++rb) {
-#pragma unroll
-          for (int t = 0; t < MT; ++t) acc2[rb][t] = f32x16{};
-          E[rb] = 1000;
-        }
+        for (int t = 0; t < MT; ++t) acc2[t] = f32x16{};
+        E = 1000;
       }
       const float* slot = ring + csl * SLOTF;
-      const FusedTile T = fused_tile(a, ctile);
-      const int gxo = T.x0 + col;
+      const int gxo = T2.x0 + col;
       const float* w2s = slot + 2 * KS * 256 + lane * 4;
-      float g[2][8];
-      const float* hwin4 = smem + (st & 1) * LF_HBUF + 4 * kh * 2 * LF_PP + 4 * (2 * cw * LF_HWD + col);
+      float g[8];
+      const float* hwin4 = smem + (st & 1) * LF_HBUF + 4 * kh * 2 * LF_PP + 4 * (wave * LF_HWD + col);
       const float* tapd = slot + (2 * KS + 2 * MT) * 256 + 4 * kh * LF_DSTR;
-      f32x4 tc[4][9], wc[4][12];
-      auto ld_taps = [&](int dd, int r) __attribute__((always_inline)) {
-#pragma unroll
-        for (int x = 0; x < 3; ++x) tc[dd][3 * r + x] = *reinterpret_cast<const f32x4*>(tapd + dd * LF_DSTR + 4 * (3 * r + x));
+      f32x4 tc[4][9], wc[4][9];
+      auto ld_stage = [&](int dd, int r) __attribute__((always_inline)) {
+#pragma unroll
+        for (int x = 0; x < 3; ++x) {
+          tc[dd][3 * r + x] = *reinterpret_cast<const f32x4*>(tapd + dd * LF_DSTR + 4 * (3 * r + x));
+          wc[dd][3 * r + x] = *reinterpret_cast<const f32x4*>(hwin4 + dd * 2 * LF_PP + 4 * (r * LF_HWD + x));
+        }
       };
-      auto ld_row = [&](int dd, int r) __attribute__((always_inline)) {
-#pragma unroll
-        for (int x = 0; x < 3; ++x)
-          wc[dd][3 * r + x] = *reinterpret_cast<const f32x4*>(hwin4 + dd * 2 * LF_PP + 4 * (r * LF_HWD + x));
-      };
-      auto gate2 = [&](const f32x4& mv, int rb, int dd) __attribute__((always_inline)) {
+      ld_stage(0, 0);
+#pragma unroll
+      for (int dd = 0; dd < 4; ++dd) {
+        f32x4 mv;
+        ld_stage(dd, 1);
+        __builtin_amdgcn_sched_barrier(0);
+        mv = lf_mul4(tc[dd][0], wc[dd][0]);
+#pragma unroll
+        for (int x = 1; x < 3; ++x) mv = lf_fma4(tc[dd][x], wc[dd][x], mv);
+        __builtin_amdgcn_sched_barrier(0);
+        ld_stage(dd, 2);
+        __builtin_amdgcn_sched_barrier(0);
+#pragma unroll
+        for (int x = 3; x < 6; ++x) mv = lf_fma4(tc[dd][x], wc[dd][x], mv);
+        __builtin_amdgcn_sched_barrier(0);
+        if (dd < 3) ld_stage(dd + 1, 0);
+        __builtin_amdgcn_sched_barrier(0);
+#pragma unroll
+        for (int x = 6; x < 9; ++x) mv = lf_fma4(tc[dd][x], wc[dd][x], mv);
 #pragma unroll
         for (int e = 0; e < 2; ++e) {
           const float m = mv[2 * e], v = mv[2 * e + 1];
-          g[rb][2 * dd + e] = (GRR_FUSED_DIAG & 8) ? (m * v) : (m * v) * __builtin_amdgcn_rcpf(1.0f + __builtin_amdgcn_exp2f(m));
-        }
-      };
-      ld_taps(0, 0);
-      ld_row(0, 0);
-      ld_row(0, 1);
-#pragma unroll
-      for (int dd = 0; dd < 4; ++dd) {
-        f32x4 mv0, mv1;
-        ld_taps(dd, 1);
-        ld_row(dd, 2);
+          g[2 * dd + e] = (GRR_FUSED_DIAG & 8) ? (m * v) : (m * v) * __builtin_amdgcn_rcpf(1.0f + __builtin_amdgcn_exp2f(m));
+        }
         __builtin_amdgcn_sched_barrier(0);
-        mv0 = tc[dd][0] * wc[dd][0];
-        mv1 = tc[dd][0] * wc[dd][3];
-#pragma unroll
-        for (int x = 1; x < 3; ++x) {
-          mv0 = __builtin_elementwise_fma(tc[dd][x], wc[dd][x], mv0);
-          mv1 = __builtin_elementwise_fma(tc[dd][x], wc[dd][3 + x], mv1);
-        }
-        __builtin_amdgcn_sched_barrier(0);
-        ld_taps(dd, 2);
-        ld_row(dd, 3);
-        __builtin_amdgcn_sched_barrier(0);
-#pragma unroll
-        for (int x = 0; x < 3; ++x) {
-          mv0 = __builtin_elementwise_fma(tc[dd][3 + x], wc[dd][3 + x], mv0);
-          mv1 = __builtin_elementwise_fma(tc[dd][3 + x], wc[dd][6 + x], mv1);
-        }
-        __builtin_amdgcn_sched_barrier(0);
-        if (dd < 3) {
-          ld_taps(dd + 1, 0);
-          ld_row(dd + 1, 0);
-          ld_row(dd + 1, 1);
-        }
-        __builtin_amdgcn_sched_barrier(0);
-#pragma unroll
-        for (int x = 0; x < 3; ++x) {
-          mv0 = __builtin_elementwise_fma(tc[dd][6 + x], wc[dd][6 + x], mv0);
-          mv1 = __builtin_elementwise_fma(tc[dd][6 + x], wc[dd][9 + x], mv1);
-        }
-        gate2(mv0, 0, dd);
-        gate2(mv1, 1, dd);
-        __builtin_amdgcn_sched_barrier(0);
-      }
-      FSTAMP(1);
+      }
+      FSTAMP(4);
+      const int yy = T2.y0 + wave;
       if (a.g) {
-        float* gb = a.g + (int64_t)T.b * hid * HW;
-#pragma unroll
-        for (int rb = 0; rb < 2; ++rb) {
-          const int yy = T.y0 + 2 * cw + rb;
-          if (yy < H && gxo < W) {
-#pragma unroll
-            for (int jj = 0; jj < 8; ++jj) {
-              const int pj = 16 * ch + 8 * kh + jj;
-              if (pj < hid) gb[(int64_t)pj * HW + yy * W + gxo] = g[rb][jj];
-            }
+        float* gb = a.g + (int64_t)T2.b * hid * HW;
+        if (yy < H && gxo < W) {
+#pragma unroll
+          for (int jj = 0; jj < 8; ++jj) {
+            const int pj = 16 * ch + 8 * kh + jj;
+            if (pj < hid) gb[(int64_t)pj * HW + yy * W + gxo] = g[jj];
           }
         }
       }
-#pragma unroll
-      for (int rb = 0; rb < 2; ++rb) {
+      {
         float gm = 0.f;
 #pragma unroll
-        for (int jj = 0; jj < 8; ++jj) gm = fmaxf(gm, fabsf(g[rb][jj]));
+        for (int jj = 0; jj < 8; ++jj) gm = fmaxf(gm, fabsf(g[jj]));
         const auto gs = __builtin_amdgcn_permlane32_swap(__float_as_uint(gm), __float_as_uint(gm), false, false);
         gm = fmaxf(__uint_as_float(gs[0]), __uint_as_float(gs[1]));
-        int eg = E[rb];
+        int eg = E;
         if (gm != 0.f) {
           int e;
           frexpf(gm, &e);
-          eg = min(E[rb], clampi(14 - e, -100, 100));
-        }
-        if (__builtin_amdgcn_readfirstlane((int)__any(eg != E[rb] && E[rb] != 1000)) != 0) {
-          const float f = E[rb] != 1000 ? ldexpf(1.0f, eg - E[rb]) : 1.0f;
-#pragma unroll
-          for (int t = 0; t < MT; ++t) acc2[rb][t] *= f;
-        }
-        E[rb] = eg;
+          eg = min(E, clampi(14 - e, -100, 100));
+        }
+        if (__builtin_amdgcn_readfirstlane((int)__any(eg != E && E != 1000)) != 0) {
+          const float f = E != 1000 ? ldexpf(1.0f, eg - E) : 1.0f;
+#pragma unroll
+          for (int t = 0; t < MT; ++t) acc2[t] *= f;
+        }
+        E = eg;
         const int Eu = eg == 1000 ? 0 : eg;
         f16x8 gh, gl;
 #pragma unroll
         for (int jj = 0; jj < 8; ++jj) {
-          const float v = ldexpf(g[rb][jj], Eu);
+          const float v = ldexpf(g[jj], Eu);
           const _Float16 h0 = (_Float16)v;
           gh[jj] = h0;
           gl[jj] = (_Float16)(v - (float)h0);
@@ -1303,97 +1317,83 @@
         for (int t = 0; t < MT; ++t) {
           const f16x8 ah = *reinterpret_cast<const f16x8*>(w2s + (2 * t + 0) * 256);
           const f16x8 al = *reinterpret_cast<const f16x8*>(w2s + (2 * t + 1) * 256);
-          acc2[rb][t] = __builtin_amdgcn_mfma_f32_32x32x16_f16(al, gh, acc2[rb][t], 0, 0, 0);
-          acc2[rb][t] = __builtin_amdgcn_mfma_f32_32x32x16_f16(ah, gl, acc2[rb][t], 0, 0, 0);
-          acc2[rb][t] = __builtin_amdgcn_mfma_f32_32x32x16_f16(ah, gh, acc2[rb][t], 0, 0, 0);
-        }
-      }
-      FSTAMP(2);
+          acc2[t] = __builtin_amdgcn_mfma_f32_32x32x16_f16(al, gh, acc2[t], 0, 0, 0);
+          acc2[t] = __builtin_amdgcn_mfma_f32_32x32x16_f16(ah, gl, acc2[t], 0, 0, 0);
+          acc2[t] = __builtin_amdgcn_mfma_f32_32x32x16_f16(ah, gh, acc2[t], 0, 0, 0);
+        }
+      }
+      __builtin_amdgcn_s_setprio(0);
+      FSTAMP(5);
       if (ch == nch - 1) {
         const float s0 = a.skip[0], s1 = a.skip[1];
         const int c8 = 8 * ((C + 7) / 8);
         const int cx = IN8 ? c8 : C, co = OUT8 ? c8 : C;
         const __amdgpu_buffer_rsrc_t xrs = __builtin_amdgcn_make_buffer_rsrc(
-            const_cast<float*>(a.x + (int64_t)T.b * cx * HW), 0, (int)((int64_t)cx * HW * 4), 0x00020000);
-        const __amdgpu_buffer_rsrc_t ors = __builtin_amdgcn_make_buffer_rsrc(a.out + (int64_t)T.b * co * HW, 0,
+            const_cast<float*>(a.x + (int64_t)T2.b * cx * HW), 0, (int)((int64_t)cx * HW * 4), 0x00020000);
+        const __amdgpu_buffer_rsrc_t ors = __builtin_amdgcn_make_buffer_rsrc(a.out + (int64_t)T2.b * co * HW, 0,
                                                                               (int)((int64_t)co * HW * 4), 0x00020000);
-        const int Eb[2] = {E[0], E[1]};
-#pragma unroll
-        for (int rb = 0; rb < 2; ++rb) {
-          const float sc = s1 * ldexpf(1.0f, Eb[rb] == 1000 ? 0 : -Eb[rb]);
-#pragma unroll
-          for (int t = 0; t < MT; ++t)
-#pragma unroll
-            for (int u = 0; u < 16; ++u) acc2[rb][t][u] *= sc * r2s[32 * t + (u & 3) + 8 * (u >> 2) + 4 * kh];
-        }
+        const float sc = s1 * ldexpf(1.0f, E == 1000 ? 0 : -E);
+#pragma unroll
+        for (int t = 0; t < MT; ++t)
+#pragma unroll
+          for (int u = 0; u < 16; ++u) acc2[t][u] *= sc * r2s[32 * t + (u & 3) + 8 * (u >> 2) + 4 * kh];
         __builtin_amdgcn_sched_barrier(0);
         int hw4 = __builtin_amdgcn_readfirstlane(HW * 4);
         asm volatile("" : "+s"(hw4));
-        uint32_t vx[2], vo[2], vx8[2], vo8[2];
-#pragma unroll
-        for (int rb = 0; rb < 2; ++rb) {
-          const int yy = T.y0 + 2 * cw + rb;
-          const uint32_t pix = (uint32_t)(min(yy, H - 1) * W + min(gxo, W - 1));
-          const bool in = yy < H && gxo < W;
-          vx[rb] = (uint32_t)(4 * kh * HW + pix) * 4u;
-          vo[rb] = in ? vx[rb] : 0x80000000u;
-          vx8[rb] = pix * 32u + 16u * kh;
-          vo8[rb] = in ? vx8[rb] : 0x80000000u;
-        }
-        float xv[2][MT][16];
-#pragma unroll
-        for (int rb = 0; rb < 2; ++rb)
-#pragma unroll
-          for (int t = 0; t < MT; ++t) {
-            if constexpr (IN8) {
-#pragma unroll
-              for (int q = 0; q < 4; ++q) {
-                const u32x4 v = __builtin_bit_cast(
-                    u32x4, __builtin_amdgcn_raw_buffer_load_b128(xrs, vx8[rb], (4 * t + q) * 8 * hw4, 0));
-#pragma unroll
-                for (int r = 0; r < 4; ++r) xv[rb][t][4 * q + r] = __uint_as_float(v[r]);
-              }
-            } else {
-#pragma unroll
-              for (int u = 0; u < 16; ++u)
-                xv[rb][t][u] = __uint_as_float(
-                    __builtin_amdgcn_raw_buffer_load_b32(xrs, vx[rb], (32 * t + (u & 3) + 8 * (u >> 2)) * hw4, 0));
+        const uint32_t pix = (uint32_t)(min(yy, H - 1) * W + min(gxo, W - 1));
+        const bool in = yy < H && gxo < W;
+        const uint32_t vx = (uint32_t)(4 * kh * HW + pix) * 4u, vo = in ? vx : 0x80000000u;
+        const uint32_t vx8 = pix * 32u + 16u * kh, vo8 = in ? vx8 : 0x80000000u;
+        float xv[MT][16];
+#pragma unroll
+        for (int t = 0; t < MT; ++t) {
+          if constexpr (IN8) {
+#pragma unroll
+            for (int q = 0; q < 4; ++q) {
+              const u32x4 v = __builtin_bit_cast(
+                  u32x4, __builtin_amdgcn_raw_buffer_load_b128(xrs, vx8, (4 * t + q) * 8 * hw4, 0));
+#pragma unroll
+              for (int r = 0; r < 4; ++r) xv[t][4 * q + r] = __uint_as_float(v[r]);
             }
+          } else {
+#pragma unroll
+            for (int u = 0; u < 16; ++u)
+              xv[t][u] = __uint_as_float(
+                  __builtin_amdgcn_raw_buffer_load_b32(xrs, vx, (32 * t + (u & 3) + 8 * (u >> 2)) * hw4, 0));
           }
-#pragma unroll
-        for (int rb = 0; rb < 2; ++rb)
-#pragma unroll
-          for (int t = 0; t < MT; ++t) {
-            if constexpr (OUT8) {
-#pragma unroll
-              for (int q = 0; q < 4; ++q) {
-                u32x4 v;
-#pragma unroll
-                for (int r = 0; r < 4; ++r) v[r] = __float_as_uint(s0 * xv[rb][t][4 * q + r] + acc2[rb][t][4 * q + r]);
-                __builtin_amdgcn_raw_buffer_store_b128(__builtin_bit_cast(decltype(__builtin_amdgcn_raw_buffer_load_b128(
-                                                           ors, 0, 0, 0)), v),
-                                                       ors, vo8[rb], (4 * t + q) * 8 * hw4, 0);
-              }
-            } else {
-#pragma unroll
-              for (int u = 0; u < 16; ++u)
-                __builtin_amdgcn_raw_buffer_store_b32(__float_as_uint(s0 * xv[rb][t][u] + acc2[rb][t][u]), ors, vo[rb],
-                                                      (32 * t + (u & 3) + 8 * (u >> 2)) * hw4, 0);
+        }
+#pragma unroll
+        for (int t = 0; t < MT; ++t)
+#pragma unroll
+          for (int u = 0; u < 16; ++u) acc2[t][u] = s0 * xv[t][u] + acc2[t][u];
+#pragma unroll
+        for (int t = 0; t < MT; ++t) {
+          if constexpr (OUT8) {
+#pragma unroll
+            for (int q = 0; q < 4; ++q) {
+              const u32x4 v{__float_as_uint(acc2[t][4 * q]), __float_as_uint(acc2[t][4 * q + 1]),
+                            __float_as_uint(acc2[t][4 * q + 2]), __float_as_uint(acc2[t][4 * q + 3])};
+              __builtin_amdgcn_raw_buffer_store_b128(__builtin_bit_cast(decltype(__builtin_amdgcn_raw_buffer_load_b128(
+                                                         ors, 0, 0, 0)), v),
+                                                     ors, vo8, (4 * t + q) * 8 * hw4, 0);
             }
+          } else {
+#pragma unroll
+            for (int u = 0; u < 16; ++u)
+              __builtin_amdgcn_raw_buffer_store_b32(__float_as_uint(acc2[t][u]), ors, vo,
+                                                    (32 * t + (u & 3) + 8 * (u >> 2)) * hw4, 0);
           }
+        }
       }
       if (++ch == nch) {
         ch = 0;
         ctile += G;
+        T2 = fused_tile(a, ctile);
       }
       csl = csl == LF_NSLOT - 1 ? 0 : csl + 1;
-    }
-    FSTAMP(3);
-    asm volatile("s_waitcnt vmcnt(0) lgkmcnt(0)" ::: "memory");
-    FSTAMP(4);
-    __builtin_amdgcn_s_barrier();
-    asm volatile("" ::: "memory");
-    FSTAMP(5);
+      FSTAMP(6);
+    }
+    if (g1_first) sync_step(i);
   }
 #if GRR_FUSED_STAMP
   stamp_out();
@@ -1617,7 +1617,7 @@
 
 grr_status lnb_forward_mfma(const float* x, const float* ln_w, const float* w1, const float* wdw, const float* w2,
                             const float* skip, float* out, float* ws, int B, int C, int hid, int H, int W,
-                            hipStream_t s, bool keep_g, int io) {
+                            hipStream_t s, bool keep_g, int io, int parts) {
   GRR_REQUIRE(io == 0 || (lnb_fused(C, hid) && !keep_g), GRR_ERR_UNSUPPORTED,
               "grr_lnb_forward_c8: the channel-blocked layout needs the fused pass (C <= 96) without the kept gate");
   if (!lnb_fused(C, hid)) {
@@ -1630,14 +1630,14 @@
   float* base = keep_g ? ws + align64((int64_t)B * hid * P) : ws;
   char* pack = reinterpret_cast<char*>(base);
   float* r2 = base + align64((int64_t)nch * fused_images(KS, MT) * 256);
-  if (g_lnb_phases & 1) {
+  if (g_lnb_phases & parts & 1) {
     const int64_t n = (int64_t)nch * fused_images(KS, MT) * 256 + C;
     hipLaunchKernelGGL(lnb_fused_pack_kernel, dim3((unsigned)std::min<int64_t>((n + 255) / 256, 4096)), dim3(256),
                        0, s, w1, ln_w, wdw, w2, pack, r2, C, hid, KS, MT, nch);
     grr_status st = launch_status("grr_lnb_forward/fused_pack");
     if (st != GRR_OK) return st;
   }
-  if (!(g_lnb_phases & 2)) return GRR_OK;
+  if (!(g_lnb_phases & parts & 2)) return GRR_OK;
   LnbFusedArgs f{};
   f.x = x; f.pack = pack; f.r2 = r2; f.skip = skip; f.out = out;
   f.g = keep_g ? ws : nullptr;
diff --git a/imagerestoration-development-unrolling_amd/kernels.py b/imagerestoration-development-unrolling_amd/kernels.py
--- a/imagerestoration-development-unrolling_amd/kernels.py
+++ b/imagerestoration-development-unrolling_amd/kernels.py
@@ -3,6 +3,7 @@
 from typing import Optional, Sequence, Tuple
 
 import os
+import weakref
 
 import torch
 
@@ -726,6 +727,31 @@
     return torch.cat(outs, 2)
 
 
+LNB_PACK_CACHE = os.environ.get("GRR_LNB_PACK_CACHE", "1") != "0"
+_LNB_PACKS = {}
+_LNB_PACKS_MAX = 256
+
+
+def _lnb_packed(dev, c: int, hid: int, ln_w: Tensor, w1: Tensor, wdw: Tensor, w2: Tensor) -> Optional[Tensor]:
+    if not LNB_PACK_CACHE or torch.is_grad_enabled() or torch.cuda.is_current_stream_capturing():
+        return None
+    ws = (ln_w, w1, wdw, w2)
+    bases = tuple(t._base if t._base is not None else t for t in ws)
+    key = tuple(id(t) for t in bases)
+    state = (tuple((t.data_ptr(), t._version) for t in ws), str(dev), c, hid)
+    hit = _LNB_PACKS.get(key)
+    if hit is not None and hit[1] == state and all(r() is t for r, t in zip(hit[0], bases)):
+        return hit[2]
+    lib = _native.load()
+    packed = torch.empty((lib.grr_lnb_fused_workspace_bytes(c, hid) + 3) // 4, dtype=torch.float32, device=dev)
+    _launch("lnb_fused_pack", 4 * packed.numel(), "grr_lnb_fused_pack", ln_w.data_ptr(), w1.data_ptr(), wdw.data_ptr(),
+            w2.data_ptr(), packed.data_ptr(), c, hid, _stream(dev))
+    if len(_LNB_PACKS) >= _LNB_PACKS_MAX:
+        _LNB_PACKS.clear()
+    _LNB_PACKS[key] = (tuple(weakref.ref(t) for t in bases), state, packed)
+    return packed
+
+
 def lnb_forward(x: Tensor, ln_w: Tensor, w1: Tensor, wdw: Tensor, w2: Tensor, skip: Tensor) -> Tensor:
     dev = _check("lnb_forward", x, ln_w, w1, wdw, w2, skip)
     b, c, h, w = x.shape
@@ -735,6 +761,12 @@
         return _lnb_banded(lambda xb: lnb_forward(xb, ln_w, w1, wdw, w2, skip), [x], h, rows)
     lib = _native.load()
     fused = bool(lib.grr_lnb_fused(c, hid))
+    packed = _lnb_packed(dev, c, hid, ln_w, w1, wdw, w2) if fused else None
+    if packed is not None:
+        out = torch.empty_like(x)
+        _launch("lnb_fused", 4 * b * h * w * 2 * c, "grr_lnb_forward_packed", x.data_ptr(), packed.data_ptr(),
+                skip.data_ptr(), out.data_ptr(), b, c, hid, h, w, 0, _stream(dev), flops=lnb_flops(b * h * w, c, c, hid))
+        return out
     nbytes = lib.grr_lnb_fused_workspace_bytes(c, hid) if fused else lib.grr_lnb_workspace_bytes(b, c, hid, h, w)
     ws = torch.empty((nbytes + 3) // 4, dtype=torch.float32, device=dev)
     out = torch.empty_like(x)
@@ -797,9 +829,15 @@
             raise ValueError("lnb_forward_c8: channels")
     hid = w2.shape[1]
     lib = _native.load()
-    ws = torch.empty((lib.grr_lnb_fused_workspace_bytes(c, hid) + 3) // 4, dtype=torch.float32, device=dev)
     out = torch.empty(c8_shape(b, c, h, w) if out_c8 else (b, c, h, w), dtype=torch.float32, device=dev)
     xc = x.contiguous()
+    packed = _lnb_packed(dev, c, hid, ln_w, w1, wdw, w2)
+    if packed is not None:
+        _launch("lnb_fused", 4 * b * h * w * 2 * c, "grr_lnb_forward_packed", xc.data_ptr(), packed.data_ptr(),
+                skip.data_ptr(), out.data_ptr(), b, c, hid, h, w, int(in_c8) | 2 * int(out_c8), _stream(dev),
+                flops=lnb_flops(b * h * w, c, c, hid))
+        return out
+    ws = torch.empty((lib.grr_lnb_fused_workspace_bytes(c, hid) + 3) // 4, dtype=torch.float32, device=dev)
     _launch("lnb_fused", 4 * b * h * w * 2 * c, "grr_lnb_forward_c8", xc.data_ptr(), ln_w.data_ptr(), w1.data_ptr(),
             wdw.data_ptr(), w2.data_ptr(), skip.data_ptr(), out.data_ptr(), ws.data_ptr(), b, c, hid, h, w,
             int(in_c8) | 2 * int(out_c8), _stream(dev), flops=lnb_flops(b * h * w, c, c, hid))
diff --git a/include/grr.h b/include/grr.h
--- a/include/grr.h
+++ b/include/grr.h
@@ -193,6 +193,10 @@
                                 int hid, int H, int W, void* stream);
 int grr_lnb_fused(int C, int hid);
 int64_t grr_lnb_fused_workspace_bytes(int C, int hid);
+grr_status grr_lnb_fused_pack(const float* ln_w, const float* w1, const float* wdw, const float* w2, void* packed,
+                              int C, int hid, void* stream);
+grr_status grr_lnb_forward_packed(const float* x, const void* packed, const float* skip, float* out, int B, int C,
+                                  int hid, int H, int W, int layout, void* stream);
 grr_status grr_lnb_set_fused(int enable);
 grr_status grr_lnb_forward_rep(const float* src, int Cs, int R, const float* x, const float* ln_w, const float* w1,
                                const float* wdw, const float* w2, const float* skip, float* out, void* workspace,
```

Result: faster. 151.8 MPix/s (median of 5 runs) (+2.5%).
